# francescobrigante/Audio-Style-Transfer

Measured on AMD Instinct MI355X. Metric: audio-seconds/sec/node (train step, 4s@22.05kHz pairs), higher is better.
Workload: dtype bf16; 1 GPU; configs[1]: batch=8 4 s clips per GPU (S=2, x=(B,S,2,287,597)), full train2 step: STFT + CQT front-end from resident waveforms, encoders+decoder+discriminator, all losses, D and G phases, grad clip, Adam; global_batch=8, parallelism=dp1, hip_graph=True, dp_semantics=per-rank BN and batch-coupled losses

## Files before the change

### audio-style-transfer_amd/ast_amd/_lib.py

```python
from __future__ import annotations

import ctypes as C
import os

import torch

_HERE = os.path.dirname(os.path.abspath(__file__))
LIB_PATH = os.environ.get("AST_HIP_LIB") or os.path.join(_HERE, "libast_hip.so")

F32, BF16 = 0, 1
MAX_TAPS = 9
IGEMM_ACCUMULATE, IGEMM_RELU, IGEMM_WS_ZEROED, IGEMM_STATS, IGEMM_BN_SUMS, IGEMM_BN_NO_RELU, IGEMM_PER_IMAGE = (1 << b for b in range(7))
IGEMM_SLOTS_SHIFT, IGEMM_DET = 8, 4096

vp, i32, i64, f32 = C.c_void_p, C.c_int32, C.c_int64, C.c_float


class Gather(C.Structure):
    _fields_ = [(n, i32) for n in ("N", "Hs", "Ws", "Cs", "Hm", "Wm", "sh", "sw", "oh", "ow", "Hd", "Wd", "Cd",
                                   "dsh", "dsw", "doh", "dow", "ntaps", "wtaps")] + [("tap", i32 * MAX_TAPS)]


class WeightDesc(C.Structure):
    _fields_ = [("w", vp), ("u", vp), ("v", vp), ("sigma", vp), ("scratch", vp), ("wf", vp), ("wb", vp)] + \
# ... 27 lines not shown
    "ast_weight_grads_flush_t": ([vp, vp, i32, vp], i32),
    "ast_dropout_fwd": ([vp, vp, vp, i64, f32, C.c_uint64, vp, vp], i32),
    "ast_weight_grad_unpack": ([vp, i32, vp, vp, vp, vp, vp, i32, i32, i32, i32, i32, i32, i32, vp, vp], i32),
    "ast_chan_stats": ([vp, vp, i32, i32, i32, i32, i32, vp], i32),
    "ast_norm_finalize": ([vp, i32, vp, i32, i32, i32, i32, i32, vp, vp, vp, vp, i32, f32, vp, vp, vp, vp, C.c_long, vp], i32),
    "ast_affine_act": ([vp, vp, vp, vp, vp, vp, vp, i32, i32, i32, i32, i32, vp], i32),
    "ast_bn_apply_fwd": ([vp, vp, vp, vp, i32, C.c_long, vp, vp, vp, vp, vp, vp, f32, vp, vp, f32, vp, vp, i32, i32, i32, i32, i32, i32, vp], i32),
    "ast_bn_apply_bwd": ([vp, vp, vp, vp, vp, vp, i32, C.c_long, vp, vp, vp, vp, vp, vp, vp, vp, vp, vp, vp, vp, vp, vp, i32, i32, i32, i32, i32, i32, vp], i32),
    "ast_norm_bwd_sums": ([vp, vp, vp, vp, vp, i32, i32, i32, i32, i32, i32, vp], i32),
    "ast_norm_bwd_sums_pre": ([vp, vp, vp, vp, vp, i32, i32, i32, i32, i32, i32, vp, vp, vp, vp, vp], i32),
    "ast_norm_bwd_apply_pre": ([vp, vp, vp, vp, vp, vp, vp, vp, i32, i32, i32, i32, i32, vp, vp, vp, vp, vp], i32),
    "ast_norm_bwd_finalize": ([vp, i32, i32, i32, i32, i32, vp, vp, vp, vp, vp, vp, vp, vp, vp, vp, vp, vp, vp], i32),
    "ast_norm_bwd_finalize_n": ([vp, i32, i32, i32, i32, i32, vp, vp, vp, vp, vp, vp, vp, vp, vp, vp, vp, vp, C.c_long, vp], i32),
    "ast_igemm_bn": ([vp, vp, vp, vp, C.POINTER(Gather), i32, i32, vp, C.c_long, vp, vp, vp, vp], i32),
    "ast_norm_bwd_apply": ([vp, vp, vp, vp, vp, vp, vp, vp, i32, i32, i32, i32, i32, vp], i32),
    "ast_layernorm_fwd": ([vp, vp, vp, vp, vp, vp, i32, i32, f32, i32, vp], i32),
    "ast_layernorm_bwd": ([vp, vp, vp, vp, vp, vp, vp, vp, i32, i32, i32, vp], i32),
    "ast_add_drop_ln_fwd": ([vp, vp, vp, vp, vp, vp, vp, vp, vp, i32, i32, f32, f32, C.c_uint64, vp, vp], i32),
    "ast_add_drop_ln_bwd": ([vp, vp, vp, vp, vp, vp, vp, vp, vp, vp, vp, i32, i32, vp], i32),
    "ast_adaptive_pool_fwd": ([vp, vp, i32, i32, i32, i32, i32, i32, i32, vp], i32),
    "ast_adaptive_pool_bwd": ([vp, vp, i32, i32, i32, i32, i32, i32, i32, vp], i32),
    "ast_bilinear_fwd": ([vp, vp, i32, i32, i32, i32, i32, i32, i32, i32, vp], i32),
    "ast_bilinear_bwd": ([vp, vp, i32, i32, i32, i32, i32, i32, i32, i32, vp], i32),
    "ast_attn_fwd": ([vp, vp, vp, vp, vp, i32, i32, i32, i32, i32, i32, i32, i32, i32, vp, vp], i32),
    "ast_attn_bwd": ([vp, vp, vp, vp, vp, vp, vp, vp, i32, i32, i32, i32, i32, i32, i32, i32, vp, vp], i32),
    "ast_rowmix": ([vp, vp, vp, i32, i32, i32, vp], i32),
    "ast_attn_fwd_p": ([vp, vp, vp, vp, vp, i32, i32, i32, i32, i32, i32, i32, i32, i32, vp, f32, C.c_uint64, vp, vp], i32),
    "ast_attn_bwd_p": ([vp, vp, vp, vp, vp, vp, vp, vp, i32, i32, i32, i32, i32, i32, i32, i32, vp, f32, C.c_uint64, vp, vp], i32),
    "ast_add": ([vp, vp, vp, i64, i32, vp], i32),
    "ast_relu_bwd": ([vp, vp, vp, i64, i32, vp], i32),
    "ast_dropout_mask": ([vp, i64, f32, C.c_uint64, vp, vp], i32),
    "ast_mul": ([vp, vp, vp, i64, i32, vp], i32),
    "ast_recon_loss": ([vp, vp, i64, i32, i32, i32, i32, f32, f32, f32, f32, f32, vp, vp, vp], i32),
    "ast_recon_loss_total": ([vp, vp, i64, i32, i32, i32, i32, C.POINTER(f32), C.POINTER(f32), vp, vp, vp, vp], i32),
    "ast_infonce": ([vp, vp, i32, i32, f32, vp, vp, vp, vp], i32),
    "ast_margin": ([vp, i32, i32, f32, vp, vp, vp], i32),
    "ast_hsic": ([vp, vp, i32, i32, vp, vp, vp, vp, vp], i32),
    "ast_crosscov": ([vp, vp, i32, i32, vp, vp, vp, vp, vp], i32),
    "ast_istft": ([vp, i32, i32, vp, vp, vp], i32),
    "ast_bin_stats_acc": ([vp, vp, vp, i32, i32, i32, vp], i32),
    "ast_zscore": ([vp, vp, vp, vp, i32, i32, i32, f32, vp], i32),
    "ast_sections_overlap_avg": ([vp, vp, i32, i32, i32, i32, i32, i32, i32, vp], i32),
    "ast_cross_entropy": ([vp, vp, i32, i32, vp, vp, vp], i32),
    "ast_softmax_entropy": ([vp, i32, i32, vp, vp, vp], i32),
    "ast_scale": ([vp, vp, f32, vp, i64, i32, vp], i32),
    "ast_colsum_acc": ([vp, i64, i32, i32, vp, i32, vp], i32),
    "ast_sumsq": ([vp, i64, vp, vp], i32),
    "ast_adam": ([vp, vp, vp, vp, i64, f32, f32, f32, f32, f32, vp, vp, f32, vp], i32),
    "ast_adam_dev": ([vp, vp, vp, vp, i64, vp, f32, f32, f32, f32, vp, vp, vp], i32),
    "ast_set_values": ([vp, C.POINTER(f32), i32, vp], i32),
    "ast_weighted_sum": ([C.POINTER(vp), C.POINTER(i32), i32, vp, vp, vp], i32),
    "ast_weighted_sum_bwd": ([vp, C.POINTER(i32), i32, vp, vp, vp], i32),
    "ast_counter_incr": ([vp, vp], i32),
    "ast_stft_sections": ([vp, i32, i32, vp, vp, vp, i32, i32, i32, i32, vp], i32),
    "ast_cqt_octaves": ([vp, vp, vp, vp, vp, vp, i32, i32, vp, vp, vp, i32, vp, i32, i32, i32, vp], i32),
    "ast_cqt_sections": ([vp, i32, i32, i32, vp, vp, vp, i32, i32, i32, i32, i32, vp], i32),
    "ast_resample_poly": ([vp, i32, i32, vp, i32, i32, i32, i32, vp, i32, f32, vp], i32),
    "ast_wgrad_rep": ([vp, vp, vp, C.POINTER(Gather), i32, i32, vp], i32),
    "ast_wgrad_slab": ([vp, vp, vp, C.POINTER(Gather), i32, i32, C.POINTER(i32), vp], i32),
    "ast_slab_sum": ([C.POINTER(vp), C.POINTER(i64), C.POINTER(i32), i32, vp], i32),
    "ast_ordered_sum": ([vp, i64, i32, i32, vp, i32, vp], i32),
    "ast_igemm_ws_floats_det": ([C.POINTER(Gather), i32], C.c_long),
    "ast_sumsq_det": ([vp, i64, vp, vp, i32, vp], i32),
    "ast_colsum_acc_det": ([vp, i64, i32, i32, vp, i32, vp, i32, vp], i32),
    "ast_chan_stats_det": ([vp, vp, i32, i32, i32, i32, vp, i32, vp], i32),
    "ast_norm_bwd_sums_det": ([vp, vp, vp, vp, vp, i32, i32, i32, i32, i32, vp, vp, vp, vp, vp, i32, vp], i32),
    "ast_layernorm_bwd_det": ([vp, vp, vp, vp, vp, vp, vp, vp, i32, i32, i32, vp, vp], i32),
    "ast_add_drop_ln_bwd_det": ([vp, vp, vp, vp, vp, vp, vp, vp, vp, vp, vp, i32, i32, vp, vp], i32),
    "ast_recon_loss_total_det": ([vp, vp, i64, i32, i32, i32, i32, C.POINTER(f32), C.POINTER(f32), vp, C.c_long, vp, vp, vp], i32),
    "ast_weight_grads_flush_det": ([vp, vp, i32, vp, C.c_long, vp], i32),
    "ast_bigk_gemm_det_ws_floats": ([i32, i32, i32], C.c_long),
    "ast_bigk_gemm_det": ([vp, vp, vp, vp, i32, i32, i32, vp, C.c_long, vp], i32),
    "ast_bign_dgrad_det_ws_floats": ([i32, i32, i32], C.c_long),
    "ast_bign_dgrad_det": ([vp, vp, vp, i32, i32, i32, i32, vp, C.c_long, vp], i32),
    "ast_skinny_gemm_wide": ([vp, vp, vp, vp, i32, i32, i32, i32, i32, i32, vp], i32),
    "ast_skinny_gemm_wide_ex": ([vp, vp, vp, vp, i32, i32, i32, i32, i32, i32, vp, vp, f32, C.c_uint64, vp, vp], i32),
    "ast_linear_wgrad_wide": ([vp, vp, vp, vp, i32, i32, i32, i32, i32, vp], i32),
    "ast_bigk_gemm_wide": ([vp, vp, vp, vp, i32, i32, i32, i32, vp], i32),
    "ast_bigk_gemm_wide_det_ws_floats": ([i32, i32, i32], C.c_long),
    "ast_bigk_gemm_wide_det": ([vp, vp, vp, vp, i32, i32, i32, vp, C.c_long, vp], i32),
    "ast_bign_dgrad_wide": ([vp, vp, vp, i32, i32, i32, i32, vp], i32),
    "ast_bign_dgrad_wide_det_ws_floats": ([i32, i32, i32], C.c_long),
    "ast_bign_dgrad_wide_det": ([vp, vp, vp, i32, i32, i32, i32, vp, C.c_long, vp], i32),
    "ast_tok_max_ops": ([], i32),
    "ast_tok_program": ([vp, i32, i32, i32, vp, vp, vp, vp], i32),
    "ast_attn_fwd_len": ([vp, vp, vp, vp, vp, i32, i32, i32, i32, i32, i32, i32, i32, i32, vp, i32, vp], i32),
    "ast_sections_overlap_avg_len": ([vp, vp, i32, i32, i32, i32, i32, i32, i32, vp, vp, vp], i32),
    "ast_istft_len": ([vp, i32, i32, vp, vp, vp, vp], i32),
    "ast_frontend_lengths": ([vp, i32, i32, i32, i32, vp, vp, vp], i32),
    "ast_frontend_lengths_host": ([i32, i32, i32, i32, C.POINTER(i32 * 4)], i32),
    "ast_stft_sections_len": ([vp, i32, i32, vp, vp, vp, i32, i32, i32, i32, vp, vp], i32),
    "ast_decimate2_len": ([vp, i32, i32, vp, i32, i32, vp, i32, f32, vp, i32, i32, i32, i32, vp], i32),
    "ast_cqt_octaves_len": ([vp, vp, vp, vp, vp, vp, i32, i32, vp, vp, vp, i32, vp, i32, i32, i32, vp, i32, i32, i32, vp], i32),
    "ast_cqt_sections_len": ([vp, i32, i32, i32, vp, vp, vp, i32, i32, i32, i32, i32, vp, i32, vp], i32),
    "ast_bign_gemm_len": ([vp, vp, vp, vp, i32, i32, i32, i32, i32, i32, vp, vp], i32),
    "ast_resample_poly_len": ([vp, i32, i32, i32, vp, i32, i32, i32, i32, vp, i32, f32, vp, vp, vp], i32),
    "ast_spec_mse_ws_floats": ([i32, i32, i32], C.c_long),
    "ast_spec_mse_len": ([vp, i32, vp, i32, i32, vp, vp, i32, vp, C.c_long, vp, vp], i32),
    "ast_band_energy_ws_floats": ([i32, i32], C.c_long),
    "ast_band_energy_len": ([vp, i32, i32, vp, i32, vp, C.c_long, vp, vp], i32),
    "ast_band_energy_run_frames": ([], i32),
    "ast_pearson_rows": ([vp, vp, i32, i32, vp, vp], i32),
    "ast_mel_table_words": ([], i32),
    "ast_mel_table": ([i32, vp], i32),
    "ast_mfcc_run_frames": ([], i32),
    "ast_mfcc_ws_floats": ([i32, i32, i32], C.c_long),
    "ast_mfcc_len": ([vp, i32, i32, vp, i32, i32, i32, vp, vp, C.c_long, vp, vp], i32),
    "ast_mfcc_distance_ws_floats": ([i32, i32, i32, i32], C.c_long),
    "ast_mfcc_distance_len": ([vp, i32, vp, i32, i32, vp, vp, i32, i32, i32, vp, vp, C.c_long, vp, vp], i32),
    "ast_onset_tile_frames": ([], i32),
    "ast_recurrence_chunk_frames": ([], i32),
    "ast_onset_strength_ws_floats": ([i32, i32], C.c_long),
    "ast_onset_strength_len": ([vp, i32, i32, vp, i32, vp, vp, C.c_long, vp, vp], i32),
    "ast_onset_detect_ws_floats": ([i32, i32], C.c_long),
    "ast_onset_detect_len": ([vp, i32, i32, vp, i32, vp, vp, C.c_long, vp, vp], i32),
    "ast_onset_accuracy_ws_floats": ([i32, i32, i32], C.c_long),
    "ast_onset_accuracy_len": ([vp, i32, vp, i32, i32, vp, vp, i32, vp, vp, C.c_long, vp, vp], i32),
    "ast_recurrence_ws_floats": ([i32, i32], C.c_long),
    "ast_recurrence_len": ([vp, i32, i32, vp, i32, vp, vp, C.c_long, vp, vp, vp], i32),
    "ast_self_similarity_distance_ws_floats": ([i32, i32, i32], C.c_long),
    "ast_self_similarity_distance_len": ([vp, i32, vp, i32, i32, vp, vp, i32, vp, vp, C.c_long, vp, vp], i32),
    "ast_frame_rms_tile_frames": ([], i32),
    "ast_mfcc_mean_chunk_frames": ([], i32),
    "ast_frame_rms_ws_floats": ([i32, i32], C.c_long),
    "ast_frame_rms_len": ([vp, i32, i32, vp, f32, i32, vp, C.c_long, vp, vp, vp, vp, vp, vp, vp], i32),
    "ast_window_sound_len": ([vp, i32, i32, vp, i32, f32, vp, vp, vp], i32),
    "ast_mfcc_mean_ws_floats": ([i32, i32, i32], C.c_long),
    "ast_mfcc_mean_len": ([vp, i32, i32, vp, i32, i32, i32, vp, vp, C.c_long, vp, vp], i32),
    "ast_gain_rows_len": ([vp, i32, i32, vp, vp, C.c_double, vp, vp], i32),
    "ast_chroma_run_frames": ([], i32),
    "ast_pitch_band": ([i32, C.POINTER(i32), C.POINTER(i32)], i32),
    "ast_tuning_debug_words": ([], i32),
    "ast_tuning_ws_floats": ([i32, i32, i32], C.c_long),
    "ast_tuning_len": ([vp, i32, i32, vp, vp, i32, i32, i32, i32, vp, C.c_long, vp, vp, vp], i32),
    "ast_chroma_len": ([vp, i32, i32, vp, vp, i32, i32, i32, i32, vp, vp, vp], i32),
    "ast_chroma_distance_ws_floats": ([i32, i32, i32], C.c_long),
    "ast_chroma_distance_len": ([vp, i32, vp, i32, i32, vp, vp, i32, vp, C.c_long, vp, vp], i32),
    "ast_chroma_similarity_ws_floats": ([i32, i32, i32], C.c_long),
    "ast_chroma_similarity_len": ([vp, i32, vp, i32, i32, vp, vp, i32, vp, C.c_long, vp, vp], i32),
    "ast_pitch_mean_len": ([vp, i32, i32, vp, vp, i32, i32, vp, vp], i32),
    "ast_pitch_correlation_ws_floats": ([i32, i32, i32], C.c_long),
    "ast_pitch_correlation_len": ([vp, i32, vp, i32, i32, vp, vp, i32, vp, C.c_long, vp, vp], i32),
    "ast_state_digest": ([C.POINTER(vp), C.POINTER(C.c_longlong), i32, vp, vp], i32),
}

EXPORTS = tuple(_SIGS) + ("ast_last_error",)

_lib = None


PROFILE_CALLS = None
NEXT_BYTES = None


def _es(dtype_code):
    return 2 if dtype_code == BF16 else 4


CALL_BYTES = {
    "ast_affine_act": lambda a: a[7] * a[8] * a[9] * _es(a[11]) * (2 + (1 if a[3] else 0)),
    "ast_norm_bwd_apply_pre": lambda a: a[8] * a[9] * a[10] * _es(a[12]) * (3 + (2 if a[3] else 0)),
    "ast_norm_bwd_sums_pre": lambda a: a[5] * a[6] * a[7] * _es(a[9]) * (2 + (1 if a[3] else 0)),
    "ast_bn_apply_fwd": lambda a: a[18] * a[19] * a[20] * _es(a[23]) * (2 + (1 if a[1] else 0)),
    "ast_bn_apply_bwd": lambda a: a[22] * a[23] * a[24] * _es(a[27]) * (3 + (2 if a[2] else 0)),
    "ast_chan_stats": lambda a: a[2] * a[3] * a[4] * _es(a[5]),
    "ast_recon_loss": lambda a: 3 * 4 * a[3] * a[4] * 2 * a[5] * a[6],
# ... 86 lines not shown
```

### audio-style-transfer_amd/ast_amd/config.py

```python
import torch

compute_dtype = torch.float32


def set_compute_dtype(dtype):
    global compute_dtype
    if dtype not in (torch.float32, torch.bfloat16):
        raise ValueError("compute dtype must be torch.float32 or torch.bfloat16")
    compute_dtype = dtype


import os as _os
fused_tokens = _os.environ.get("AST_FUSED_TOKENS", "1") != "0"
tok_programs = int(_os.environ.get("AST_TOK_PROGRAMS", "0"))

fused_bn_stats = _os.environ.get("AST_FUSED_BN_STATS", "1") != "0"

bn_mask_from_preact = _os.environ.get("AST_BN_MASK_FROM_PREACT", "1") != "0"

fused_bn_bwd = _os.environ.get("AST_FUSED_BN_BWD", "1") != "0"

wgrad_replicas = int(_os.environ.get("AST_WGRAD_REPLICAS", "8"))

fused_finalize = _os.environ.get("AST_FUSED_FINALIZE", "0") != "0"

wgrad_slabs = int(_os.environ.get("AST_WGRAD_SLABS", "0"))

wgrad_defer = _os.environ.get("AST_WGRAD_DEFER", "1") != "0"
wgrad_defer_streams = int(_os.environ.get("AST_WGRAD_DEFER_STREAMS", "1"))
wgrad_defer_pool = _os.environ.get("AST_WGRAD_DEFER_POOL", "0") != "0"
wgrad_defer_lend = float(_os.environ.get("AST_WGRAD_DEFER_LEND", "1.0"))

deterministic = _os.environ.get("AST_DETERMINISTIC", "0") not in ("", "0")


def check_deterministic_supported(flag, world=1):
    if not flag:
        return
    if tok_programs != 0:
        raise ValueError("deterministic mode: the token programs (AST_TOK_PROGRAMS != 0) add floats with atomics; set AST_TOK_PROGRAMS=0")
    if world > 1:
        raise ValueError("deterministic mode covers one GPU (world == 1); data parallelism is not supported")


def set_deterministic(flag):
    global deterministic
    flag = bool(flag)
    check_deterministic_supported(flag)
    deterministic = flag
```

### audio-style-transfer_amd/ast_amd/decoder_trunk.py

```python
from __future__ import annotations

import torch
import torch.nn as nn

from . import layers as L
from . import config, ops, tokprog
from ._lib import len_tensor
from .style_encoder import SinusoidalPositionalEncoding, _module_bank


def bank_linear(bank, lin: nn.Linear):
    return bank.add(lin.weight, "linear", L.tok_dtype, bias=lin.bias)


class DecoderTrunk(nn.Module):
    token_programs = False

    decode_mode = "recompute"

    def _build_trunk(self, d_model, nhead, num_layers, dim_feedforward, dropout):
        self.d_model = d_model
        self.content_proj = nn.Linear(d_model, d_model)
        self.class_proj = nn.Linear(d_model, d_model)
        self.pos_encoding = SinusoidalPositionalEncoding(d_model)
        layer = nn.TransformerDecoderLayer(d_model=d_model, nhead=nhead, dim_feedforward=dim_feedforward, dropout=dropout,
                                           batch_first=True, norm_first=True)
        self.transformer_decoder = nn.TransformerDecoder(layer, num_layers=num_layers)
        self.start_token = nn.Parameter(torch.randn(1, 1, d_model))
        self.input_norm = nn.LayerNorm(d_model)
        self.output_norm = nn.LayerNorm(d_model)
        self.dropout = nn.Dropout(dropout)

    def _init_weights(self):
        for name, p in self.named_parameters():
            if "weight" in name:
                nn.init.xavier_uniform_(p, gain=0.2) if p.dim() > 1 else nn.init.zeros_(p)
            elif "bias" in name:
                nn.init.zeros_(p)

    def register(self, bank):
        self._cp, self._kp = bank_linear(bank, self.content_proj), bank_linear(bank, self.class_proj)
        self._layers = [L.DecoderLayer(bank, l) for l in self.transformer_decoder.layers]

    def _prepare(self):
        _module_bank(self).prepare(self.training)

    def _check_lengths(self, lengths, B):
        len_tensor(lengths, B, "lengths", training=self.training)

    def _memory(self, content_emb, class_emb):
        B, Sc, D = content_emb.shape
        if 2 * Sc > ops.ATTN_MAX_L:
            raise ValueError(f"{Sc} content sections make {2 * Sc} memory tokens; the attention core takes {ops.ATTN_MAX_L} "
                             f"(at most {ops.ATTN_MAX_L // 2} sections per clip)")
        cm = L.linear(content_emb.reshape(B * Sc, D), self._cp).view(B, Sc, D)
        km = L.linear(class_emb, self._kp).unsqueeze(1).expand(-1, Sc, -1)
        return ops.dropout(torch.cat([cm, km], dim=1), self.dropout.p, self.training)

    def prepare_memory(self, content_emb, class_emb, lengths=None):
        self._check_lengths(lengths, content_emb.shape[0])
        self._prepare()
        return self._memory(content_emb, class_emb)

    def _stack(self, tgt, memory, lengths=None):
        if (self.token_programs and lengths is None and config.tok_programs > 0
                and tokprog.decoder_stack_ok(tgt, memory, self._layers)):
            return tokprog.decoder_stack(tgt, memory, self._layers, self.training)
        for lyr in self._layers:
            tgt = lyr(tgt, memory, self.training, lengths)
        return tgt

    def _teacher_forced(self, emb, memory):
        tgt = torch.cat([self.start_token.expand(emb.shape[0], 1, -1), emb[:, :-1, :]], dim=1)
        tgt = L.layer_norm(self.pos_encoding(tgt), self.input_norm)
        return self._generate(self._stack(tgt, memory), None)

    def forward_training(self, y, memory):
        self._prepare()
        return self._training_pass(y, memory)

    def _inference_pass_cached(self, memory, target_length, lengths=None):
        B = memory.size(0)
        mem_kv = [lyr.memory_kv(memory) for lyr in self._layers]
        caches = [None] * len(self._layers)
        tok = self.start_token.expand(B, -1, -1)
        pe = self.pos_encoding.pe
        outs = []
        for t in range(target_length):
            x = tok + pe[:, t:t + 1]
            for i, lyr in enumerate(self._layers):
                x, caches[i] = lyr.step(x, caches[i], mem_kv[i], lengths)
            outs.append(x)
            tok = x
        return self._generate(torch.cat(outs, dim=1), lengths)

    def _inference_pass(self, memory, target_length=None, lengths=None):
        B = memory.size(0)
        if target_length is None:
            target_length = memory.size(1) // 2
        if target_length > self.pos_encoding.pe.size(1):
            raise ValueError(f"target_length {target_length}, but the positional table holds {self.pos_encoding.pe.size(1)} positions")
        if self.decode_mode == "kv_cache" and not torch.is_grad_enabled():
            return self._inference_pass_cached(memory, target_length, lengths)
        seq = self.start_token.expand(B, -1, -1)
        outs = []
        for _ in range(target_length):
            nxt = self._stack(self.pos_encoding(seq), memory, lengths)[:, -1:, :]
            outs.append(nxt)
            seq = torch.cat([seq, nxt], dim=1)
        return self._generate(torch.cat(outs, dim=1), lengths)

    def forward_inference(self, memory, target_length=None, lengths=None):
        self._check_lengths(lengths, memory.size(0))
        self._prepare()
        return self._inference_pass(memory, target_length, lengths)
```

### audio-style-transfer_amd/ast_amd/layers.py

```python
from __future__ import annotations

import contextlib
import ctypes as C
import os

import torch
import torch.nn as nn

from . import config, ops, streams
from ._lib import LinWg, WeightDesc, check, dcode, lib, ptr, stream
from .ops import PackedWeight, pad8


class WeightBank:

    def __init__(self):
        self.specs = []
        self.entries: list[PackedWeight] = []
        self._key = None
        self._keys = {}
        self._flush_pending = False
        self._flush_stream = None
        self._lin_deferred = []
        self._pinned = []
# ... 353 lines not shown
    return _bn_apply(x, bn, training, relu, stats)


def conv_with_stats(x, pw, k, stride, pad, training):
    stats = None
    if training and config.fused_bn_stats:
        N, H, W, Cs = x.shape
        g, _ = ops.gather_direct(N, H, W, Cs, pw.Cop, k, stride, pad)
        if ops.stats_fusable(g, ops.dcode(x.dtype)):
            stats = ops.stat_table(ops.stat_slots(pw.Cop) * pw.Cop * 2, x.device)
    return ops.Conv2dFn.apply(x, pw.weight, pw, k, stride, pad, False, stats, _link_of(x)), stats


def convT_bn_act(x, pw, k, stride, pad, out_pad, bn: nn.BatchNorm2d, training, relu=True):
    stats = None
    if training and config.fused_bn_stats:
        N, H, W, Cs = x.shape
        Ho = (H - 1) * stride - 2 * pad + k + out_pad
        Wo = (W - 1) * stride - 2 * pad + k + out_pad
        gs = ops.gathers_transposed(N, H, W, Cs, Ho, Wo, pw.Cop, k, stride, pad)
        if all(ops.stats_fusable(g, ops.dcode(x.dtype)) for g in gs):
            stats = ops.stat_table(ops.stat_slots(pw.Cop) * pw.Cop * 2, x.device)
    y = ops.ConvT2dFn.apply(x, pw.weight, pw, k, stride, pad, out_pad, False, stats, _link_of(x))
    return _bn_apply(y, bn, training, relu, stats)


def res_head(x, p1, pd, stride, training):
    stats = None
    if training and config.fused_bn_stats:
        N, H, W, Cs = x.shape
        g, _ = ops.gather_direct(N, H, W, Cs, p1.Cop, 3, stride, 1)
        if ops.stats_fusable(g, ops.dcode(x.dtype)):
            stats = ops.stat_table(ops.stat_slots(p1.Cop) * p1.Cop * 2, x.device)
    in_stats = None
    if training and config.fused_bn_stats:
        N, H, W, Cs = x.shape
        gd, _ = ops.gather_direct(N, H, W, Cs, pd.Cop, 1, stride, 0)
        if ops.in_stats_fusable(gd, ops.dcode(x.dtype)):
            in_stats = ops.stat_table(N * pd.Cop * 2, x.device)
    c1, idn = ops.ResHeadFn.apply(x, p1.weight, pd.weight, p1, pd, stride, stats, in_stats)
    return c1, idn, stats, in_stats


def conv_bn_act(x, pw, k, stride, pad, bn: nn.BatchNorm2d, training, relu=True):
    y, stats = conv_with_stats(x, pw, k, stride, pad, training)
    return _bn_apply(y, bn, training, relu, stats)


def layer_norm(x, ln: nn.LayerNorm):
    return ops.LayerNormFn.apply(x, ln.weight, ln.bias, ln.eps)


class MHA:

    def __init__(self, bank: WeightBank, m: nn.MultiheadAttention, cross: bool):
        d = m.embed_dim
        self.m, self.d, self.h, self.cross = m, d, m.num_heads, cross
        if cross:
            self.q = bank.add(m.in_proj_weight, "linear", tok_dtype, bias=m.in_proj_bias, rows=(0, d))
            self.kv = bank.add(m.in_proj_weight, "linear", tok_dtype, bias=m.in_proj_bias, rows=(d, 3 * d))
        else:
            self.qkv = bank.add(m.in_proj_weight, "linear", tok_dtype, bias=m.in_proj_bias)
        self.out = bank.add(m.out_proj.weight, "linear", tok_dtype, bias=m.out_proj.bias)

    def __call__(self, x, mem, training, p_drop, causal=False, key_mask=None):
        B, Lq, d = x.shape
        dh = d // self.h
        if self.cross:
            Lk = mem.shape[1]
            q = linear(x.reshape(B * Lq, d), self.q)
            kv = linear(mem.reshape(B * Lk, d), self.kv)
            k_off, v_off = 0, d
        else:
            Lk = Lq
            q = kv = linear(x.reshape(B * Lq, d), self.qkv)
            k_off, v_off = d, 2 * d
        if key_mask is not None:
            ops.require_inference(q, kv)
        o = ops.AttnCoreFn.apply(q, kv, B, self.h, Lq, Lk, dh, k_off, v_off, causal, float(p_drop) if training else 0.0,
                                 *(key_mask or ()))
        return linear(o, self.out).view(B, Lq, d)


class EncoderLayer:

    def __init__(self, bank, layer: nn.TransformerEncoderLayer):
        self.l = layer
        self.attn = MHA(bank, layer.self_attn, cross=False)
        self.ff1 = bank.add(layer.linear1.weight, "linear", tok_dtype, bias=layer.linear1.bias)
        self.ff2 = bank.add(layer.linear2.weight, "linear", tok_dtype, bias=layer.linear2.bias)

    def __call__(self, x, training, lengths=None):
        l, p = self.l, self.l.dropout.p
        B, L, d = x.shape
        km = None if lengths is None else (lengths, L)
        if not config.fused_tokens:
            x = layer_norm(x + ops.dropout(self.attn(x, None, training, l.self_attn.dropout, key_mask=km), l.dropout1.p, training),
                           l.norm1)
            h = ops.dropout(linear(x.reshape(B * L, d), self.ff1, relu=True), p, training)
            h = ops.dropout(linear(h, self.ff2), l.dropout2.p, training).view(B, L, d)
            return layer_norm(x + h, l.norm2)
        _, x = ops.add_drop_ln(x, self.attn(x, None, training, l.self_attn.dropout, key_mask=km), l.norm1, l.dropout1.p, training)
        h = ops.ffn(x.reshape(B * L, d), self.ff1, self.ff2, p, training)
        _, y = ops.add_drop_ln(x, h.view(B, L, d), l.norm2, l.dropout2.p, training)
        return y


class DecoderLayer:

    def __init__(self, bank, layer: nn.TransformerDecoderLayer):
        self.l = layer
        self.sa = MHA(bank, layer.self_attn, cross=False)
        self.ca = MHA(bank, layer.multihead_attn, cross=True)
        self.ff1 = bank.add(layer.linear1.weight, "linear", tok_dtype, bias=layer.linear1.bias)
        self.ff2 = bank.add(layer.linear2.weight, "linear", tok_dtype, bias=layer.linear2.bias)

    def __call__(self, x, memory, training, lengths=None):
        l = self.l
        B, L, d = x.shape
        km = None if lengths is None else (lengths, memory.shape[1] // 2)
        if not config.fused_tokens:
            h = layer_norm(x, l.norm1)
            x = x + ops.dropout(self.sa(h, None, training, l.self_attn.dropout, causal=True), l.dropout1.p, training)
            h = layer_norm(x, l.norm2)
            x = x + ops.dropout(self.ca(h, memory, training, l.multihead_attn.dropout, key_mask=km), l.dropout2.p, training)
            h = layer_norm(x, l.norm3)
            h = ops.dropout(linear(h.reshape(B * L, d), self.ff1, relu=True), l.dropout.p, training)
            h = ops.dropout(linear(h, self.ff2), l.dropout3.p, training).view(B, L, d)
            return x + h
        h = layer_norm(x, l.norm1)
        x, h = ops.add_drop_ln(x, self.sa(h, None, training, l.self_attn.dropout, causal=True), l.norm2, l.dropout1.p, training)
        x, h = ops.add_drop_ln(x, self.ca(h, memory, training, l.multihead_attn.dropout, key_mask=km), l.norm3, l.dropout2.p, training)
        h = ops.ffn(h.reshape(B * L, d), self.ff1, self.ff2, l.dropout.p, training)
        x, _ = ops.add_drop_ln(x, h.view(B, L, d), None, l.dropout3.p, training)
        return x

    def memory_kv(self, memory):
        B, Lm, d = memory.shape
        return linear(memory.reshape(B * Lm, d), self.ca.kv), Lm

    def step(self, x_t, kv_self, mem_kv, lengths=None):
        l = self.l
        B, _, d = x_t.shape
        dh = d // self.sa.h
        h = layer_norm(x_t, l.norm1).reshape(B, d)
        qkv = linear(h, self.sa.qkv)
        new_kv = qkv[:, d:].reshape(B, 1, 2 * d)
        kv_self = new_kv if kv_self is None else torch.cat([kv_self, new_kv], dim=1)
        t1 = kv_self.shape[1]
        q = qkv[:, :d].contiguous()
        o = ops.AttnCoreFn.apply(q, kv_self.reshape(B * t1, 2 * d), B, self.sa.h, 1, t1, dh, 0, d, False, 0.0)
        x = x_t.reshape(B, d) + linear(o, self.sa.out)
        h = layer_norm(x, l.norm2)
        kvm, Lm = mem_kv
        qm = linear(h, self.ca.q)
        if lengths is not None:
            ops.require_inference(qm, kvm)
        o = ops.AttnCoreFn.apply(qm, kvm, B, self.ca.h, 1, Lm, dh, 0, d, False, 0.0, *(() if lengths is None else (lengths, Lm // 2)))
        x = x + linear(o, self.ca.out)
        h = layer_norm(x, l.norm3)
        x = x + linear(linear(h, self.ff1, relu=True), self.ff2)
        return x.view(B, 1, d), kv_self
```

### audio-style-transfer_amd/ast_amd/ops.py

```python
from __future__ import annotations

import ctypes
import functools
import math

import torch

from . import _lib, config
from ._lib import Gather, check, dcode, len_tensor, lib, ptr, stream


@functools.lru_cache(maxsize=None)
def const_tensor(values, dtype, device):
    return torch.tensor(values, dtype=dtype, device=device)


def pad8(c: int) -> int:
    return (c + 7) // 8 * 8


def _tap(dh, dw, wt):
    return (dh + 64) | ((dw + 64) << 8) | (wt << 16)


# ... 313 lines not shown
        _igemm(x, pwd.wf, pwd.bias_ptr_tensor(), idn, gd, stats=in_stats, per_image=in_stats is not None)
        ctx.save_for_backward(x)
        ctx.pws, ctx.geoms, ctx.stride = (pw1, pwd), (g1, gd), stride
        return c1, idn

    @staticmethod
    def backward(ctx, dc1, didn):
        (x,) = ctx.saved_tensors
        (pw1, pwd), (g1, gd), stride = ctx.pws, ctx.geoms, ctx.stride
        dc1, didn = dc1.contiguous(), didn.contiguous()
        N, H, W, Cs = x.shape
        if pw1.dwp is None or pwd.dwp is None:
            raise RuntimeError("weights were prepared in eval/no-grad mode; run the forward in training mode before backward")
        _wgrad(dc1, x, pw1.dwp, g1, pw1.replicas, pw1)
        _wgrad(didn, x, pwd.dwp, gd, pwd.replicas, pwd)
        pw1.bank.request_flush()
        dx = None
        if ctx.needs_input_grad[0]:
            dx = torch.empty_like(x)
            Ho, Wo = dc1.shape[1], dc1.shape[2]
            for g in gathers_transposed(N, Ho, Wo, pw1.Cop, H, W, Cs, 3, stride, 1):
                _igemm(dc1, pw1.wb, None, dx, g)
            for g in gathers_transposed(N, Ho, Wo, pwd.Cop, H, W, Cs, 1, stride, 0):
                if g.ntaps > 0:
                    _igemm(didn, pwd.wb, None, dx, g, flags=_lib.IGEMM_ACCUMULATE)
        return dx, None, None, None, None, None, None, None


class ConvT2dFn(torch.autograd.Function):

    @staticmethod
    def forward(ctx, x, weight, pw: PackedWeight, k, stride, pad, out_pad, bias_grad, stats=None, link=None):
        N, H, W, Cs = x.shape
        Ho = (H - 1) * stride - 2 * pad + k + out_pad
        Wo = (W - 1) * stride - 2 * pad + k + out_pad
        y = torch.empty((N, Ho, Wo, pw.Cop), dtype=x.dtype, device=x.device)
        b = pw.bias_ptr_tensor()
        for g in gathers_transposed(N, H, W, Cs, Ho, Wo, pw.Cop, k, stride, pad):
            _igemm(x, pw.wf, b, y, g, stats=stats)
        ctx.save_for_backward(x)
        ctx.pw, ctx.args, ctx.bias_grad, ctx.link = pw, (k, stride, pad, Ho, Wo), bias_grad, link
        return y

    @staticmethod
    def backward(ctx, dy):
        (x,) = ctx.saved_tensors
        pw, (k, stride, pad, Ho, Wo) = ctx.pw, ctx.args
        dy = dy.contiguous()
        N, H, W, Cs = x.shape
        g, (Hx, Wx) = gather_direct(N, Ho, Wo, pw.Cop, Cs, k, stride, pad)
        assert (Hx, Wx) == (H, W), "ConvTranspose2d geometry mismatch"
        if pw.dwp is None:
            raise RuntimeError("weights were prepared in eval/no-grad mode; run the forward in training mode before backward")
        _wgrad(x, dy, pw.dwp, g, pw.replicas, pw)
        pw.bank.request_flush()
        if ctx.bias_grad:
            pw.add_bias_grad(dy)
        dx = None
        if ctx.needs_input_grad[0]:
            dx = torch.empty_like(x)
            link = _bn_link_ready(ctx.link, (g,), x)
            _igemm(dy, pw.wb, None, dx, g, bn=link)
            if link is not None:
                link.filled = True
        return dx, None, None, None, None, None, None, None, None, None


SKINNY_MAX_ROWS = 64
WIDE_MAX_ROWS = 1024
ATTN_MAX_L = 1024


def _token_entry(who, stem, rows, tail=""):
    if rows > WIDE_MAX_ROWS:
        raise RuntimeError(f"{who}: {rows} token rows > {WIDE_MAX_ROWS} (the cap of the wide token path, AST_WIDE_MAX_ROWS)")
    return f"ast_{stem}{'' if rows <= SKINNY_MAX_ROWS else '_wide'}{tail}"


def _token_call(who, stem, rows, tail, *args):
    name = _token_entry(who, stem, rows, tail)
    check(getattr(lib(), name)(*args, stream()), name)


def _token_rows_ok(rows):
    return rows <= SKINNY_MAX_ROWS or (config.deterministic and rows <= WIDE_MAX_ROWS)


class LinearFn(torch.autograd.Function):

    @staticmethod
    def forward(ctx, x, weight, pw: PackedWeight, relu):
        x = x.contiguous()
        rows = x.shape[0]
        assert x.shape[1] == pw.Cip and x.dtype == pw.dtype, (x.shape, pw.Cip, x.dtype, pw.dtype)
        ctx.skinny = (_token_rows_ok(rows) and pw.KK == 1 and pw.u is None and pw.Ci == pw.Cip
                      and (rows <= SKINNY_MAX_ROWS or x.dtype == torch.float32))
        y = torch.empty((rows, pw.Cop), dtype=x.dtype, device=x.device)
        if ctx.skinny:
            if pw.Cop != pw.Co:
                y.zero_()
            b = None if pw.bias is None else pw.bias.data_ptr() + 4 * pw.b_off
            _token_call("LinearFn", "skinny_gemm", rows, "", ptr(x), pw.weight.data_ptr() + 4 * pw.w_off, b, ptr(y), rows, pw.Co, pw.Ci, pw.s_co, pw.Cop, int(relu))
        else:
            g, _ = gather_direct(rows, 1, 1, pw.Cip, pw.Cop, 1, 1, 0)
            _igemm(x, pw.wf, pw.bias_ptr_tensor(), y, g, _lib.IGEMM_RELU if relu else 0)
        ctx.save_for_backward(x, y if relu else None)
        ctx.pw, ctx.relu = pw, relu
        return y

    @staticmethod
    def backward(ctx, dy):
        x, y = ctx.saved_tensors
        pw = ctx.pw
        dy = dy.contiguous()
        rows = x.shape[0]
        if ctx.relu:
            dz = torch.empty_like(dy)
            check(lib().ast_relu_bwd(ptr(dy), ptr(y), ptr(dz), dy.numel(), dcode(dy.dtype), stream()), "ast_relu_bwd")
            dy = dz
        dx = None
        if ctx.skinny:
            if pw.bank is not None:
                pw.bank.defer_linear_wgrad(pw, dy, x)
            else:
                gw = acc_grad(pw.weight)
                gb = None if pw.bias is None else acc_grad(pw.bias).data_ptr() + 4 * pw.b_off
                _token_call("LinearFn", "linear_wgrad", rows, "", ptr(dy), ptr(x), gw.data_ptr() + 4 * pw.w_off, gb, rows, pw.Co, pw.Ci, pw.Cop, pw.s_co)
            if ctx.needs_input_grad[0]:
                dx = torch.empty_like(x)
                _token_call("LinearFn", "skinny_gemm", rows, "", ptr(dy), ptr(pw.wb), None, ptr(dx), rows, pw.Ci, pw.Cop, pw.Cop, pw.Cip, 0)
            return dx, None, None, None
        if config.deterministic:
            raise RuntimeError(f"LinearFn: the non-skinny weight gradient (> {WIDE_MAX_ROWS} token rows, spectral norm, unpadded channels "
                               "or bf16 above 64 rows) has no deterministic form")
        g, _ = gather_direct(rows, 1, 1, pw.Cip, pw.Cop, 1, 1, 0)
        dwp = torch.zeros((pw.Cop, 1, pw.Cip), dtype=torch.float32, device=x.device)
        _wgrad(dy, x, dwp, g)
        pw.add_weight_grad(dwp, 0)
        pw.add_bias_grad(dy)
        if ctx.needs_input_grad[0]:
            gb, _ = gather_direct(rows, 1, 1, pw.Cop, pw.Cip, 1, 1, 0)
            dx = torch.empty_like(x)
            _igemm(dy, pw.wb, None, dx, gb)
        return dx, None, None, None


class BigLinearFn(torch.autograd.Function):

    @staticmethod
    def forward(ctx, x, weight, bias):
        x = x.contiguous()
        rows, K = x.shape
        N = weight.shape[0]
        assert weight.shape[1] == K and x.dtype == torch.float32 and weight.is_contiguous()
        ctx.big_in = K > N
        stem, tail = ("bigk_gemm", "_det" if config.deterministic else "") if ctx.big_in else ("skinny_gemm", "")
        _token_entry("BigLinearFn", stem, rows, tail)
        y = torch.empty((rows, N), dtype=torch.float32, device=x.device)
        if tail:
            ws = det_ws(getattr(lib(), _token_entry("BigLinearFn", stem, rows, "_det_ws_floats"))(rows, N, K), x.device)
            _token_call("BigLinearFn", stem, rows, tail, ptr(x), ptr(weight), ptr(bias), ptr(y), rows, N, K, ptr(ws), ws.numel())
        elif ctx.big_in:
            _token_call("BigLinearFn", stem, rows, tail, ptr(x), ptr(weight), ptr(bias), ptr(y), rows, N, K, N)
        else:
            _token_call("BigLinearFn", stem, rows, tail, ptr(x), ptr(weight), ptr(bias), ptr(y), rows, N, K, K, N, 0)
        ctx.save_for_backward(x)
        ctx.weight, ctx.bias = weight, bias
        return y

    @staticmethod
    def backward(ctx, dy):
        (x,) = ctx.saved_tensors
        w, b = ctx.weight, ctx.bias
        dy = dy.contiguous()
        rows, K = x.shape
        N = w.shape[0]
        _token_call("BigLinearFn", "linear_wgrad", rows, "", ptr(dy), ptr(x), ptr(acc_grad(w)), ptr(acc_grad(b)) if b is not None else None, rows, N, K, N, K)
        dx = None
        if ctx.needs_input_grad[0]:
            if ctx.big_in:
                raise NotImplementedError("BigLinearFn: input gradient of the huge-input linear (its input is data on the reference's path)")
            dx = torch.empty_like(x)
            if config.deterministic:
                ws = det_ws(getattr(lib(), _token_entry("BigLinearFn", "bign_dgrad", rows, "_det_ws_floats"))(rows, N, K), x.device)
                _token_call("BigLinearFn", "bign_dgrad", rows, "_det", ptr(dy), ptr(w), ptr(dx), rows, N, K, N, ptr(ws), ws.numel())
            else:
                _token_call("BigLinearFn", "bign_dgrad", rows, "", ptr(dy), ptr(w), ptr(dx), rows, N, K, N)
        return dx, None, None


BIGN_MAX_ROWS = 4096


def big_out_linear(x, weight, bias, S, lengths=None):
    if torch.is_grad_enabled() and any(t is not None and t.requires_grad for t in (x, weight, bias)):
        raise RuntimeError("the length-masked output linear (big_out_linear) is inference only: it has no backward; "
                           "run it under torch.no_grad()")
    x = x.contiguous()
    rows, K = x.shape
    N = weight.shape[0]
    assert weight.shape[1] == K and x.dtype == torch.float32 and weight.dtype == torch.float32 and weight.is_contiguous()
    if rows > BIGN_MAX_ROWS:
        raise RuntimeError(f"big_out_linear: {rows} rows > {BIGN_MAX_ROWS} (AST_BIGN_MAX_ROWS)")
    if S < 1 or rows % S:
        raise ValueError(f"big_out_linear: {rows} rows are not a whole number of clips of {S} sections")
    lengths = len_tensor(lengths, rows // S, "lengths", contiguous=True)
    y = torch.empty((rows, N), dtype=torch.float32, device=x.device)
    check(lib().ast_bign_gemm_len(ptr(x), ptr(weight), ptr(bias), ptr(y), rows, N, K, K, N, int(S), ptr(lengths), stream()),
          "ast_bign_gemm_len")
    return y


class FFNFn(torch.autograd.Function):

    @staticmethod
    def forward(ctx, x, w1, w2, pw1: PackedWeight, pw2: PackedWeight, p):
        x = x.contiguous()
        rows = x.shape[0]
        h = torch.empty((rows, pw1.Cop), dtype=x.dtype, device=x.device)
        y = torch.empty((rows, pw2.Cop), dtype=x.dtype, device=x.device)
        mask, seed, ctr = None, 0, None
        if p > 0.0:
            if _DropState.counter is None or _DropState.counter.device != x.device:
                _DropState.counter = torch.zeros(1, dtype=torch.int64, device=x.device)
            _DropState.calls += 1
            seed, ctr = _DropState.seed + 7919 * _DropState.calls, _DropState.counter
            mask = torch.empty_like(h)
        _token_call("FFNFn", "skinny_gemm", rows, "_ex", ptr(x), pw1.weight.data_ptr() + 4 * pw1.w_off, pw1.bias.data_ptr() + 4 * pw1.b_off, ptr(h),
                                                 rows, pw1.Co, pw1.Ci, pw1.s_co, pw1.Cop, 1, None, ptr(mask), float(p), seed, ptr(ctr))
        _token_call("FFNFn", "skinny_gemm", rows, "", ptr(h), pw2.weight.data_ptr() + 4 * pw2.w_off, pw2.bias.data_ptr() + 4 * pw2.b_off, ptr(y),
                                          rows, pw2.Co, pw2.Ci, pw2.s_co, pw2.Cop, 0)
        ctx.save_for_backward(x, h, mask)
        ctx.pw1, ctx.pw2 = pw1, pw2
        return y

    @staticmethod
    def backward(ctx, dy):
        x, h, mask = ctx.saved_tensors
        pw1, pw2 = ctx.pw1, ctx.pw2
        dy = dy.contiguous()
        rows = x.shape[0]
        pw2.bank.defer_linear_wgrad(pw2, dy, h)
        dh = torch.empty_like(h)
        if mask is None:
            _token_call("FFNFn", "skinny_gemm", rows, "", ptr(dy), ptr(pw2.wb), None, ptr(dh), rows, pw2.Ci, pw2.Cop, pw2.Cop, pw2.Cip, 0)
            dz = torch.empty_like(dh)
            check(lib().ast_relu_bwd(ptr(dh), ptr(h), ptr(dz), dh.numel(), dcode(dh.dtype), stream()), "ast_relu_bwd")
            dh = dz
        else:
            _token_call("FFNFn", "skinny_gemm", rows, "_ex", ptr(dy), ptr(pw2.wb), None, ptr(dh), rows, pw2.Ci, pw2.Cop, pw2.Cop, pw2.Cip, 0, ptr(mask), None,
                                                     0.0, 0, None)
        pw1.bank.defer_linear_wgrad(pw1, dh, x)
        dx = None
        if ctx.needs_input_grad[0]:
            dx = torch.empty_like(x)
            _token_call("FFNFn", "skinny_gemm", rows, "", ptr(dh), ptr(pw1.wb), None, ptr(dx), rows, pw1.Ci, pw1.Cop, pw1.Cop, pw1.Cip, 0)
        return dx, None, None, None, None, None


def _skinny_ok(pw, rows):
    return (_token_rows_ok(rows) and pw.KK == 1 and pw.u is None and pw.Ci == pw.Cip and pw.Co == pw.Cop and pw.bank is not None
            and pw.bias is not None)


def ffn(x2d, pw1, pw2, p, training):
    rows = x2d.shape[0]
    if _skinny_ok(pw1, rows) and _skinny_ok(pw2, rows) and x2d.dtype == torch.float32:
        return FFNFn.apply(x2d, pw1.weight, pw2.weight, pw1, pw2, float(p) if training else 0.0)
    h = dropout(LinearFn.apply(x2d, pw1.weight, pw1, True), p, training)
    h = h if pw1.Cop == pw1.Co else h[:, :pw1.Co]
    y = LinearFn.apply(h, pw2.weight, pw2, False)
    return y if pw2.Cop == pw2.Co else y[:, :pw2.Co]


_scratch = {}


def _clean_scratch(n, device, tag=None):
    key = (n, device, torch.cuda.current_stream(device).cuda_stream, tag)
    t = _scratch.get(key)
    if t is None:
        t = _scratch[key] = torch.zeros(n, dtype=torch.float32, device=device)
    return t


def det_slots(rows, per=1):
    return max(1, min(512 // per, (int(rows) + 255) // 256))


def det_ws(n, device):
    return _clean_scratch(max(1, int(n)), device, tag="det")


def _stats(x):
    N, H, W, C = x.shape
    sums = stat_table(N * C * 2, x.device)
    if config.deterministic:
        ns = det_slots(H * W, N)
        check(lib().ast_chan_stats_det(ptr(x), ptr(sums), N, H * W, C, dcode(x.dtype), ptr(det_ws(N * ns * C * 2, x.device)), ns, stream()),
              "ast_chan_stats_det")
        return sums
    check(lib().ast_chan_stats(ptr(x), ptr(sums), N, H * W, C, dcode(x.dtype), 1, stream()), "ast_chan_stats")
    return sums


def _bwd_sums(dy, y, x, r, sums3, N, HW, C, relu, dt, scale1, shift1, scale2, shift2):
    y, r, scale1, shift1, scale2, shift2 = (t if (t is None or isinstance(t, int)) else ptr(t) for t in (y, r, scale1, shift1, scale2, shift2))
    if config.deterministic:
        ns = det_slots(HW, N)
        check(lib().ast_norm_bwd_sums_det(ptr(dy), y, ptr(x), r, ptr(sums3), N, HW, C, int(relu), dt, scale1, shift1,
                                          scale2, shift2, ptr(det_ws(N * ns * C * 3, dy.device)), ns, stream()), "ast_norm_bwd_sums_det")
        return
    check(lib().ast_norm_bwd_sums_pre(ptr(dy), y, ptr(x), r, ptr(sums3), N, HW, C, int(relu), dt, 1,
                                      scale1, shift1, scale2, shift2, stream()), "ast_norm_bwd_sums")


class _SyncBN:
    world = 1
    group = None
    active = False


def set_sync_bn(world=1, group=None, force=False):
    _SyncBN.world, _SyncBN.group = int(world), group
    _SyncBN.active = _SyncBN.world > 1 or bool(force)


def _global_sums(sums, n_floats):
    import torch.distributed as dist
    g = sums[:n_floats].clone()
    dist.all_reduce(g, op=dist.ReduceOp.SUM, group=_SyncBN.group)
    return g


def _bn_batch_stats(x, gamma, beta, bn, stats=None):
    N, H, W, C = x.shape
    rows = stats.numel() // (2 * C) if stats is not None else N
    sums = stats if stats is not None else _stats(x)
    pixels = N * H * W
# ... 111 lines not shown
        N, H, W, C = c2.shape
        Creal = g1.numel()
        ctx.fused = bool(training and config.fused_finalize and not _SyncBN.active)
        if ctx.fused:
            tab1 = stats if stats is not None else _stats(c2)
            tab2 = in_stats if in_stats is not None else _stats(ds)
            rows1 = tab1.numel() // (2 * C)
            out1 = torch.empty((4, C), dtype=torch.float32, device=c2.device)
            out2 = torch.empty((4, N * C), dtype=torch.float32, device=c2.device)
            y = torch.empty_like(c2)
            check(lib().ast_bn_apply_fwd(ptr(c2), ptr(ds), ptr(y), ptr(tab1), rows1, N * H * W, ptr(tab2), ptr(g1), ptr(b1), ptr(bn.running_mean),
                                         ptr(bn.running_var), ptr(bn.num_batches_tracked), bn.eps, ptr(g2), ptr(b2), inn.eps, ptr(out1), ptr(out2),
                                         N, H * W, C, Creal, 1, dcode(c2.dtype), stream()), "ast_bn_apply_fwd")
            ctx.save_for_backward(c2, ds, None, out1[0], out1[1], out2[0], out2[1], out1[2], out1[3], out2[2], out2[3])
            ctx.params, ctx.training = (g1, b1, g2, b2), training
            return y
        if training:
            m1, r1, s1, f1 = _bn_batch_stats(c2, g1, b1, bn, stats)
        else:
            m1, r1, s1, f1 = _finalize(None, N, H * W, C, Creal, False, g1, b1, bn.running_mean, bn.running_var,
                                       True, bn.eps, c2.device)
        m2, r2, s2, f2 = _finalize(in_stats if in_stats is not None else _stats(ds), N, H * W, C, Creal, True, g2, b2, None, None, False,
                                   inn.eps, c2.device)
        y = torch.empty_like(c2)
        check(lib().ast_affine_act(ptr(c2), ptr(s1), ptr(f1), ptr(ds), ptr(s2), ptr(f2), ptr(y), N, H * W, C, 1,
                                   dcode(c2.dtype), stream()), "ast_affine_act")
        ctx.save_for_backward(c2, ds, y, m1, r1, m2, r2, s1, f1, s2, f2)
        ctx.params, ctx.training = (g1, b1, g2, b2), training
        return y

    @staticmethod
    def backward(ctx, dy):
        c2, ds, y, m1, r1, m2, r2, s1, f1, s2, f2 = ctx.saved_tensors
        pre = config.bn_mask_from_preact
        if not ctx.training:
            raise RuntimeError("ResTailFn: backward in eval mode is not on the reference's path")
        g1, b1, g2, b2 = ctx.params
        dy = dy.contiguous()
        N, H, W, C = c2.shape
        dev = c2.device
        if ctx.fused:
            tab3 = stat_table(N * C * 3, dev)
            _bwd_sums(dy, None, c2, ds, tab3, N, H * W, C, 1, dcode(c2.dtype), s1, f1, s2, f2)
            dc2, dds = torch.empty_like(c2), torch.empty_like(ds)
            check(lib().ast_bn_apply_bwd(ptr(dy), ptr(c2), ptr(ds), ptr(dc2), ptr(dds), ptr(tab3), N, N * H * W, ptr(g1), ptr(m1), ptr(r1),
                                         ptr(acc_grad(g1)), ptr(acc_grad(b1)), ptr(g2), ptr(m2), ptr(r2), ptr(acc_grad(g2)), ptr(acc_grad(b2)),
                                         ptr(s1), ptr(f1), ptr(s2), ptr(f2), N, H * W, C, g1.numel(), 1, dcode(c2.dtype), stream()), "ast_bn_apply_bwd")
            return dc2, dds, None, None, None, None, None, None, None, None, None
        sums3 = _clean_scratch(N * C * 3, dev)
        coef = (ptr(s1), ptr(f1), ptr(s2), ptr(f2)) if pre else (None, None, None, None)
        _bwd_sums(dy, y, c2, ds, sums3, N, H * W, C, 1, dcode(c2.dtype), *coef)
        k1 = torch.empty((C, 3), dtype=torch.float32, device=dev)
        k2 = torch.empty((N, C, 3), dtype=torch.float32, device=dev)
        gsum = _global_sums(sums3, N * C * 3) if _SyncBN.active else None
        check(lib().ast_norm_bwd_finalize(ptr(sums3), 1, N, H * W, C, g1.numel(), ptr(g1), ptr(m1), ptr(r1),
                                          ptr(acc_grad(g1)), ptr(acc_grad(b1)), ptr(k1), ptr(g2), ptr(m2), ptr(r2),
                                          ptr(acc_grad(g2)), ptr(acc_grad(b2)), ptr(k2), stream()),
              "ast_norm_bwd_finalize")
        if gsum is not None:
            check(lib().ast_norm_bwd_finalize(ptr(gsum), 0, N, H * W * _SyncBN.world, C, g1.numel(), ptr(g1), ptr(m1), ptr(r1),
                                              None, None, ptr(k1), None, None, None, None, None, None, stream()), "ast_norm_bwd_finalize")
        dc2, dds = torch.empty_like(c2), torch.empty_like(ds)
        check(lib().ast_norm_bwd_apply_pre(ptr(dy), ptr(y), ptr(c2), ptr(ds), ptr(k1), ptr(k2), ptr(dc2), ptr(dds), N, H * W,
                                           C, 1, dcode(c2.dtype), *coef, stream()), "ast_norm_bwd_apply")
        return dc2, dds, None, None, None, None, None, None, None, None, None


class LayerNormFn(torch.autograd.Function):
    @staticmethod
    def forward(ctx, x, gamma, beta, eps):
        shape = x.shape
        x2 = x.contiguous().view(-1, shape[-1])
        rows, D = x2.shape
        y = torch.empty_like(x2)
        mean = torch.empty(rows, dtype=torch.float32, device=x.device)
        rstd = torch.empty_like(mean)
        check(lib().ast_layernorm_fwd(ptr(x2), ptr(gamma), ptr(beta), ptr(y), ptr(mean), ptr(rstd), rows, D, eps,
                                      dcode(x2.dtype), stream()), "ast_layernorm_fwd")
        ctx.save_for_backward(x2, mean, rstd)
        ctx.gamma, ctx.beta, ctx.shape = gamma, beta, shape
        return y.view(shape)

    @staticmethod
    def backward(ctx, dy):
        x2, mean, rstd = ctx.saved_tensors
        rows, D = x2.shape
        dy2 = dy.contiguous().view(rows, D)
        dx = torch.empty_like(x2)
        if config.deterministic:
            check(lib().ast_layernorm_bwd_det(ptr(dy2), ptr(x2), ptr(ctx.gamma), ptr(mean), ptr(rstd), ptr(dx), ptr(acc_grad(ctx.gamma)),
                                              ptr(acc_grad(ctx.beta)), rows, D, dcode(x2.dtype), ptr(det_ws(2 * rows * D, dx.device)),
                                              stream()), "ast_layernorm_bwd_det")
            return dx.view(ctx.shape), None, None, None
        check(lib().ast_layernorm_bwd(ptr(dy2), ptr(x2), ptr(ctx.gamma), ptr(mean), ptr(rstd), ptr(dx),
                                      ptr(acc_grad(ctx.gamma)), ptr(acc_grad(ctx.beta)), rows, D, dcode(x2.dtype),
                                      stream()), "ast_layernorm_bwd")
        return dx.view(ctx.shape), None, None, None


class AddDropLNFn(torch.autograd.Function):

    @staticmethod
    def forward(ctx, x, sub, ln, p):
        ctx.set_materialize_grads(False)
        shape = sub.shape
        D = shape[-1]
        sub2 = sub.contiguous().view(-1, D)
        x2 = x.contiguous().view(-1, D) if x is not None else None
        rows = sub2.shape[0]
        s = torch.empty_like(sub2)
        mask = torch.empty_like(sub2) if p > 0.0 else None
        seed = 0
        if p > 0.0:
            if _DropState.counter is None or _DropState.counter.device != sub.device:
                _DropState.counter = torch.zeros(1, dtype=torch.int64, device=sub.device)
            _DropState.calls += 1
            seed = _DropState.seed + 7919 * _DropState.calls
        y = mean = rstd = None
        if ln is not None:
            y = torch.empty_like(sub2)
            mean = torch.empty(rows, dtype=torch.float32, device=sub.device)
            rstd = torch.empty_like(mean)
        check(lib().ast_add_drop_ln_fwd(ptr(x2), ptr(sub2), ptr(mask), ptr(s), ptr(ln.weight) if ln is not None else None,
                                        ptr(ln.bias) if ln is not None else None, ptr(y), ptr(mean), ptr(rstd), rows, D,
                                        float(ln.eps) if ln is not None else 0.0, float(p), seed,
                                        ptr(_DropState.counter) if p > 0.0 else None, stream()), "ast_add_drop_ln_fwd")
        ctx.save_for_backward(s, mean, rstd, mask)
        ctx.ln, ctx.shape, ctx.has_x = ln, shape, x is not None
        if ln is None:
            return s.view(shape)
        return s.view(shape), y.view(shape)

    @staticmethod
    def backward(ctx, ds_ext, dy=None):
        s, mean, rstd, mask = ctx.saved_tensors
        rows, D = s.shape
        if ds_ext is None and dy is None:
            return None, None, None, None
        ds2 = ds_ext.contiguous().view(rows, D) if ds_ext is not None else None
        dy2 = dy.contiguous().view(rows, D) if dy is not None else None
        want_dx = ctx.has_x and ctx.needs_input_grad[0]
        dx = None if (not want_dx or dy2 is None) else torch.empty_like(s)
        if dy2 is None and mask is None:
            return (ds_ext if want_dx else None), ds_ext, None, None
        dsub = torch.empty_like(s)
        ln = ctx.ln
        if config.deterministic:
            check(lib().ast_add_drop_ln_bwd_det(ptr(dy2), ptr(ds2), ptr(s), ptr(ln.weight) if dy2 is not None else None, ptr(mean),
                                                ptr(rstd), ptr(mask), ptr(dx), ptr(dsub),
                                                ptr(acc_grad(ln.weight)) if dy2 is not None else None,
                                                ptr(acc_grad(ln.bias)) if dy2 is not None else None, rows, D,
                                                ptr(det_ws(2 * rows * D, dsub.device)), stream()), "ast_add_drop_ln_bwd_det")
        else:
            check(lib().ast_add_drop_ln_bwd(ptr(dy2), ptr(ds2), ptr(s), ptr(ln.weight) if dy2 is not None else None, ptr(mean), ptr(rstd),
                                            ptr(mask), ptr(dx), ptr(dsub), ptr(acc_grad(ln.weight)) if dy2 is not None else None,
                                            ptr(acc_grad(ln.bias)) if dy2 is not None else None, rows, D, stream()), "ast_add_drop_ln_bwd")
        if want_dx and dx is None:
            dx = ds2
        return (dx.view(ctx.shape) if want_dx else None), dsub.view(ctx.shape), None, None


def add_drop_ln(x, sub, ln, p, training):
    out = AddDropLNFn.apply(x, sub, ln, float(p) if training else 0.0)
    return (out, None) if ln is None else out


class RowMixFn(torch.autograd.Function):

    @staticmethod
    def forward(ctx, x, A, At):
        x = x.contiguous()
        R_out, R_in = A.shape
        assert x.shape[0] == R_in and x.dtype == torch.float32
        y = torch.empty((R_out, x.shape[1]), dtype=torch.float32, device=x.device)
        check(lib().ast_rowmix(ptr(A), ptr(x), ptr(y), R_out, R_in, x.shape[1], stream()), "ast_rowmix")
        ctx.At = At
        return y

    @staticmethod
# ... 441 lines not shown
```

### audio-style-transfer_amd/csrc/ast_common.h

```cpp
#pragma once
#include <hip/hip_runtime.h>
#include <stdint.h>
#include <stdio.h>
#include <stdlib.h>
#include <string.h>
#include <algorithm>
#include <atomic>
#include <initializer_list>

typedef __bf16 bf16_t;
typedef __attribute__((ext_vector_type(8))) __bf16 bf16x8;
typedef __attribute__((ext_vector_type(4))) __bf16 bf16x4;
typedef __attribute__((ext_vector_type(4))) float f32x4;
typedef __attribute__((ext_vector_type(2))) float f32x2;

enum { AST_F32 = 0, AST_BF16 = 1 };

void ast_set_error(const char* fmt, ...);
#define AST_FAIL(...) do { ast_set_error(__VA_ARGS__); return -1; } while (0)
#define AST_CHECK_LAUNCH() do { hipError_t e_ = hipGetLastError(); \
    if (e_ != hipSuccess) { ast_set_error("%s:%d launch failed: %s", __FILE__, __LINE__, hipGetErrorString(e_)); return -2; } } while (0)
#define AST_HIP(x) do { hipError_t e_ = (x); \
    if (e_ != hipSuccess) { ast_set_error("%s:%d %s: %s", __FILE__, __LINE__, #x, hipGetErrorString(e_)); return -3; } } while (0)

// ... 10 lines not shown
    for (const void* k : kernels) AST_HIP(hipFuncSetAttribute(k, hipFuncAttributeMaxDynamicSharedMemorySize, bytes));
    if (tracked) done[dev].store(true, std::memory_order_release);
    return 0;
  }
};

template <typename T> struct U8;
template <> struct U8<float> {
  static __device__ __forceinline__ void load(const float* p, float (&v)[8]) {
    f32x4 a = *reinterpret_cast<const f32x4*>(p);
    f32x4 b = *reinterpret_cast<const f32x4*>(p + 4);
#pragma unroll
    for (int i = 0; i < 4; ++i) { v[i] = a[i]; v[4 + i] = b[i]; }
  }
  static __device__ __forceinline__ void store(float* p, const float (&v)[8]) {
    f32x4 a, b;
#pragma unroll
    for (int i = 0; i < 4; ++i) { a[i] = v[i]; b[i] = v[4 + i]; }
    *reinterpret_cast<f32x4*>(p) = a;
    *reinterpret_cast<f32x4*>(p + 4) = b;
  }
};
template <> struct U8<bf16_t> {
  static __device__ __forceinline__ void load(const bf16_t* p, float (&v)[8]) {
    bf16x8 a = *reinterpret_cast<const bf16x8*>(p);
#pragma unroll
    for (int i = 0; i < 8; ++i) v[i] = (float)a[i];
  }
  static __device__ __forceinline__ void store(bf16_t* p, const float (&v)[8]) {
    bf16x8 a;
#pragma unroll
    for (int i = 0; i < 8; ++i) a[i] = (bf16_t)v[i];
    *reinterpret_cast<bf16x8*>(p) = a;
  }
};

template <int CTRL>
__device__ __forceinline__ float dpp_mov(float v) {
  return __builtin_bit_cast(float, __builtin_amdgcn_update_dpp(0, __builtin_bit_cast(int, v), CTRL, 0xF, 0xF, false));
}
__device__ __forceinline__ float row16_sum(float v) {
  v += dpp_mov<0xB1>(v);
  v += dpp_mov<0x4E>(v);
  v += dpp_mov<0x124>(v);
  v += dpp_mov<0x128>(v);
  return v;
}
__device__ __forceinline__ float row16_transpose_sum(const float (&v)[16], const int l) {
  float w[8], x[4], y[2];
  const bool b0 = l & 1, b1 = l & 2, b2 = l & 4, b3 = l & 8;
#pragma unroll
  for (int k = 0; k < 8; ++k) w[k] = (b0 ? v[2 * k + 1] : v[2 * k]) + dpp_mov<0xB1>(b0 ? v[2 * k] : v[2 * k + 1]);
#pragma unroll
  for (int k = 0; k < 4; ++k) x[k] = (b1 ? w[2 * k + 1] : w[2 * k]) + dpp_mov<0x4E>(b1 ? w[2 * k] : w[2 * k + 1]);
#pragma unroll
  for (int k = 0; k < 2; ++k) {
    const float send = b2 ? x[2 * k] : x[2 * k + 1];
    const float lo = dpp_mov<0x124>(send), hi = dpp_mov<0x12C>(send);
    y[k] = (b2 ? x[2 * k + 1] : x[2 * k]) + (b2 ? lo : hi);
  }
  return (b3 ? y[1] : y[0]) + dpp_mov<0x128>(b3 ? y[0] : y[1]);
}
__device__ __forceinline__ float wave_sum_dpp(float v) {
  v = row16_sum(v);
  const int i = __builtin_bit_cast(int, v);
  return (__builtin_bit_cast(float, __builtin_amdgcn_readlane(i, 0)) + __builtin_bit_cast(float, __builtin_amdgcn_readlane(i, 16))) +
         (__builtin_bit_cast(float, __builtin_amdgcn_readlane(i, 32)) + __builtin_bit_cast(float, __builtin_amdgcn_readlane(i, 48)));
}
#ifdef AST_WAVE_SUM_SHFL
__device__ __forceinline__ float wave_sum(float v) {
#pragma unroll
  for (int o = 32; o > 0; o >>= 1) v += __shfl_xor(v, o, 64);
  return v;
}
#else
__device__ __forceinline__ float wave_sum(float v) { return wave_sum_dpp(v); }
#endif
__device__ __forceinline__ float wave_max(float v) {
#pragma unroll
  for (int o = 32; o > 0; o >>= 1) v = fmaxf(v, __shfl_xor(v, o, 64));
  return v;
}

__device__ __forceinline__ uint64_t mix64(uint64_t z) {
  z += 0x9E3779B97F4A7C15ull; z = (z ^ (z >> 30)) * 0xBF58476D1CE4E5B9ull; z = (z ^ (z >> 27)) * 0x94D049BB133111EBull; return z ^ (z >> 31);
}
__device__ __forceinline__ float dropout_keep(uint64_t base, uint64_t i, float p, float keep) {
  const uint32_t r = (uint32_t)(mix64(base + i) >> 40);
  return ((float)r * (1.f / 16777216.f)) >= p ? keep : 0.f;
}

__device__ __forceinline__ float block_sum(float v, float* red ) {
  v = wave_sum(v);
  const int w = threadIdx.x >> 6, nw = (blockDim.x + 63) >> 6;
  __syncthreads();
  if ((threadIdx.x & 63) == 0) red[w] = v;
  __syncthreads();
  if (threadIdx.x == 0) { float s = 0.f; for (int i = 0; i < nw; ++i) s += red[i]; red[16] = s; }
  __syncthreads();
  return red[16];
}

#define AST_DISPATCH_T(dtype, ...) \
  do { if ((dtype) == AST_F32) { using T = float; __VA_ARGS__; } \
       else if ((dtype) == AST_BF16) { using T = bf16_t; __VA_ARGS__; } \
       else AST_FAIL("%s: bad dtype %d", __func__, (int)(dtype)); } while (0)

#define AST_HIDDEN __attribute__((visibility("hidden")))
AST_HIDDEN int attn_long_fwd_launch(const float* q, const float* k, const float* v, float* o, float* probs, int B, int H, int Lq, int Lk,
                                    int dh, int ldq, int ldk, int ldo, int causal, const float* drop_mask, float p, uint64_t seed,
                                    const int64_t* d_offset, void* stream);
AST_HIDDEN int attn_long_fwd_len_launch(const float* q, const float* k, const float* v, float* o, float* probs, int B, int H, int Lq,
                                        int Lk, int dh, int ldq, int ldk, int ldo, int causal, const int32_t* key_len, int key_period,
                                        void* stream);
AST_HIDDEN int attn_long_bwd_launch(const float* dout, const float* q, const float* k, const float* v, const float* probs, float* dq,
                                    float* dk, float* dv, int B, int H, int Lq, int Lk, int dh, int ldq, int ldk, int ldo,
                                    const float* drop_mask, float p, uint64_t seed, const int64_t* d_offset, void* stream);
```

### audio-style-transfer_amd/csrc/norm.hip

```cpp
#include "ast_common.h"
#include "../../include/ast_hip.h"

namespace {

template <typename T, int MODE, bool DET = false>
__global__ __launch_bounds__(256) void chan_reduce_kernel(const T* __restrict__ a, const T* __restrict__ b,
                                                           const T* __restrict__ c, const T* __restrict__ d,
                                                           float* __restrict__ sums, int HW, int C, int ppb, int relu,
                                                           const float* __restrict__ sc1, const float* __restrict__ sf1,
                                                           const float* __restrict__ sc2, const float* __restrict__ sf2) {
  constexpr int K = MODE == 0 ? 2 : 3;
  __shared__ float red[256 * 8];
  const int U = C >> 3;
  const int PL = 256 / U;
  const int tid = threadIdx.x;
  const int u = tid % U, pl = tid / U;
  const int n = blockIdx.y;
  const int p0 = blockIdx.x * ppb, p1 = min(HW, p0 + ppb);
  float s[K][8];
#pragma unroll
  for (int k = 0; k < K; ++k)
#pragma unroll
    for (int i = 0; i < 8; ++i) s[k][i] = 0.f;
  float a1[8], b1[8], a2[8], b2[8];
// ... 418 lines not shown
            dg += (float)((double)rstd2[iq] * ((double)t2 - (double)mean2[iq] * (double)t0));
            db += t0;
          }
          if (dgamma2) dgamma2[c] += dg;
          if (dbeta2) dbeta2[c] += db;
        }
      } else { kc[3 * C + c * 3] = kc[3 * C + c * 3 + 1] = kc[3 * C + c * 3 + 2] = 0.f; }
    }
  }
  __syncthreads();

  const int U = C >> 3;
  const size_t per_img = (size_t)HW * U, base = (size_t)n * per_img;
  const size_t stride = (size_t)gridDim.x * 256;
  const bool hoist = (256 % U) == 0;
  const bool remask = relu != 0;
  float a1[8], b1[8], a2[8], b2[8];
  f32x4 kaq[6], kbq[6];
  auto load_coef = [&](int u) __attribute__((always_inline)) {
    if (remask) {
      U8<float>::load(sc1 + u * 8, a1);
      U8<float>::load(sf1 + u * 8, b1);
      if (r) {
        U8<float>::load(sc2 + (size_t)n * C + u * 8, a2);
        U8<float>::load(sf2 + (size_t)n * C + u * 8, b2);
      }
    }
    const f32x4* ka4 = reinterpret_cast<const f32x4*>(kc + u * 24);
    const f32x4* kb4 = reinterpret_cast<const f32x4*>(kc + 3 * C + u * 24);
#pragma unroll
    for (int q = 0; q < 6; ++q) { kaq[q] = ka4[q]; kbq[q] = dr ? kb4[q] : f32x4{0.f, 0.f, 0.f, 0.f}; }
  };
#define KA(k, q) kaq[((k) * 3 + (q)) >> 2][((k) * 3 + (q)) & 3]
#define KB(k, q) kbq[((k) * 3 + (q)) >> 2][((k) * 3 + (q)) & 3]
  const size_t j0 = (size_t)blockIdx.x * 256 + tid;
  if (hoist) load_coef((int)(j0 % U));
  for (size_t j = j0; j < per_img; j += stride) {
    if (!hoist) load_coef((int)(j % U));
    const size_t i = base + j;
    float dz[8], v[8], o[8], vr[8];
    U8<T>::load(dy + i * 8, dz);
    U8<T>::load(x + i * 8, v);
    if (r) U8<T>::load(r + i * 8, vr);
    if (remask) {
      float pre[8];
#pragma unroll
      for (int k = 0; k < 8; ++k) pre[k] = __builtin_fmaf(v[k], a1[k], b1[k]);
      if (r) {
#pragma unroll
        for (int k = 0; k < 8; ++k) pre[k] += __builtin_fmaf(vr[k], a2[k], b2[k]);
      }
#pragma unroll
      for (int k = 0; k < 8; ++k) dz[k] = pre[k] > 0.f ? dz[k] : 0.f;
    }
#pragma unroll
    for (int k = 0; k < 8; ++k) o[k] = KA(k, 0) * dz[k] + KA(k, 1) * v[k] + KA(k, 2);
    U8<T>::store(dx + i * 8, o);
    if (dr) {
#pragma unroll
      for (int k = 0; k < 8; ++k) o[k] = KB(k, 0) * dz[k] + KB(k, 1) * vr[k] + KB(k, 2);
      U8<T>::store(dr + i * 8, o);
    }
  }
#undef KA
#undef KB
}

__global__ void layernorm_fwd_kernel(const float* __restrict__ x, const float* __restrict__ gamma,
                                     const float* __restrict__ beta, float* __restrict__ y, float* __restrict__ mean,
                                     float* __restrict__ rstd, int rows, int D, float eps) {
  const int row = blockIdx.x * (blockDim.x >> 6) + (threadIdx.x >> 6), lane = threadIdx.x & 63;
  if (row >= rows) return;
  const float* xr = x + (size_t)row * D;
  float s = 0.f;
  for (int i = lane; i < D; i += 64) s += xr[i];
  const float m = wave_sum(s) / D;
  float q = 0.f;
  for (int i = lane; i < D; i += 64) { const float d = xr[i] - m; q += d * d; }
  const float r = rsqrtf(wave_sum(q) / D + eps);
  for (int i = lane; i < D; i += 64) y[(size_t)row * D + i] = (xr[i] - m) * r * gamma[i] + beta[i];
  if (lane == 0) { mean[row] = m; rstd[row] = r; }
}

template <bool DET = false>
__global__ void layernorm_bwd_kernel(const float* __restrict__ dy, const float* __restrict__ x,
                                     const float* __restrict__ gamma, const float* __restrict__ mean,
                                     const float* __restrict__ rstd, float* __restrict__ dx, float* dgamma, float* dbeta,
                                     int rows, int D) {
  const int row = blockIdx.x * (blockDim.x >> 6) + (threadIdx.x >> 6), lane = threadIdx.x & 63;
  if (row >= rows) return;
  const float m = mean[row], r = rstd[row];
  const float* xr = x + (size_t)row * D;
  const float* dr = dy + (size_t)row * D;
  float a = 0.f, b = 0.f;
  for (int i = lane; i < D; i += 64) {
    const float xh = (xr[i] - m) * r, g = dr[i] * gamma[i];
    a += g; b += g * xh;
  }
  a = wave_sum(a) / D; b = wave_sum(b) / D;
  for (int i = lane; i < D; i += 64) {
    const float xh = (xr[i] - m) * r, g = dr[i] * gamma[i];
    dx[(size_t)row * D + i] = r * (g - a - xh * b);
    if constexpr (DET) {
      if (dgamma) dgamma[(size_t)row * D + i] = dr[i] * xh;
      if (dbeta) dbeta[(size_t)row * D + i] = dr[i];
    } else {
      if (dgamma) unsafeAtomicAdd(dgamma + i, dr[i] * xh);
      if (dbeta) unsafeAtomicAdd(dbeta + i, dr[i]);
    }
  }
}


__global__ void add_drop_ln_fwd_kernel(const float* __restrict__ x, const float* __restrict__ sub, float* __restrict__ mask,
                                       float* __restrict__ s_out, const float* __restrict__ gamma, const float* __restrict__ beta,
                                       float* __restrict__ y, float* __restrict__ mean, float* __restrict__ rstd, int rows, int D,
                                       float eps, float p, uint64_t seed, const int64_t* __restrict__ d_offset) {
  const int row = blockIdx.x * (blockDim.x >> 6) + (threadIdx.x >> 6), lane = threadIdx.x & 63;
  if (row >= rows) return;
  const size_t o = (size_t)row * D;
  const uint64_t base = p > 0.f ? mix64(seed ^ mix64((uint64_t)(d_offset ? *d_offset : 0))) : 0;
  const float keep = 1.f / (1.f - p);
  float acc = 0.f;
  for (int i = lane; i < D; i += 64) {
    float v = sub[o + i];
    if (p > 0.f) { const float m = dropout_keep(base, o + i, p, keep); mask[o + i] = m; v *= m; }
    if (x) v += x[o + i];
    s_out[o + i] = v;
    acc += v;
  }
  if (!gamma) return;
  const float m = wave_sum(acc) / D;
  float q = 0.f;
  for (int i = lane; i < D; i += 64) { const float d = s_out[o + i] - m; q += d * d; }
  const float r = rsqrtf(wave_sum(q) / D + eps);
  for (int i = lane; i < D; i += 64) y[o + i] = (s_out[o + i] - m) * r * gamma[i] + beta[i];
  if (lane == 0) { mean[row] = m; rstd[row] = r; }
}

template <bool DET = false>
__global__ void add_drop_ln_bwd_kernel(const float* __restrict__ dy, const float* __restrict__ ds_ext, const float* __restrict__ s,
                                       const float* __restrict__ gamma, const float* __restrict__ mean, const float* __restrict__ rstd,
                                       const float* __restrict__ mask, float* __restrict__ dx, float* __restrict__ dsub,
                                       float* dgamma, float* dbeta, int rows, int D) {
  const int row = blockIdx.x * (blockDim.x >> 6) + (threadIdx.x >> 6), lane = threadIdx.x & 63;
  if (row >= rows) return;
  const size_t o = (size_t)row * D;
  float a = 0.f, b = 0.f, m = 0.f, r = 0.f;
  if (dy) {
    m = mean[row]; r = rstd[row];
    for (int i = lane; i < D; i += 64) {
      const float xh = (s[o + i] - m) * r, g = dy[o + i] * gamma[i];
      a += g; b += g * xh;
    }
    a = wave_sum(a) / D; b = wave_sum(b) / D;
  }
  for (int i = lane; i < D; i += 64) {
    float d = ds_ext ? ds_ext[o + i] : 0.f;
    if (dy) {
      const float xh = (s[o + i] - m) * r, g = dy[o + i] * gamma[i];
      d += r * (g - a - xh * b);
      if constexpr (DET) {
        if (dgamma) dgamma[o + i] = dy[o + i] * xh;
        if (dbeta) dbeta[o + i] = dy[o + i];
      } else {
        if (dgamma) unsafeAtomicAdd(dgamma + i, dy[o + i] * xh);
        if (dbeta) unsafeAtomicAdd(dbeta + i, dy[o + i]);
      }
    }
    if (dx) dx[o + i] = d;
    dsub[o + i] = mask ? d * mask[o + i] : d;
  }
}

__global__ __launch_bounds__(256) void add_drop_ln_fwd256_kernel(const float* __restrict__ x, const float* __restrict__ sub,
                                                                 float* __restrict__ mask, float* __restrict__ s_out,
                                                                 const float* __restrict__ gamma, const float* __restrict__ beta,
                                                                 float* __restrict__ y, float* __restrict__ mean, float* __restrict__ rstd,
                                                                 int rows, float eps, float p, uint64_t seed,
                                                                 const int64_t* __restrict__ d_offset) {
  constexpr int D = 256;
  const int row = blockIdx.x * 4 + (threadIdx.x >> 6), lane = threadIdx.x & 63;
  if (row >= rows) return;
  const size_t o = (size_t)row * D + lane * 4;
  const f32x4 z = {0.f, 0.f, 0.f, 0.f};
  const f32x4 sv = *reinterpret_cast<const f32x4*>(sub + o);
  const f32x4 xv = x ? *reinterpret_cast<const f32x4*>(x + o) : z;
  const f32x4 g4 = gamma ? *reinterpret_cast<const f32x4*>(gamma + lane * 4) : z;
  const f32x4 b4 = gamma ? *reinterpret_cast<const f32x4*>(beta + lane * 4) : z;
  const uint64_t base = p > 0.f ? mix64(seed ^ mix64((uint64_t)(d_offset ? *d_offset : 0))) : 0;
  __builtin_amdgcn_sched_barrier(0);
  const float keep = 1.f / (1.f - p);
  f32x4 sv2 = sv;
  if (p > 0.f) {
    f32x4 m4;
#pragma unroll
    for (int e = 0; e < 4; ++e) { m4[e] = dropout_keep(base, o + e, p, keep); sv2[e] *= m4[e]; }
    *reinterpret_cast<f32x4*>(mask + o) = m4;
  }
  f32x4 s4;
#pragma unroll
  for (int e = 0; e < 4; ++e) s4[e] = x ? sv2[e] + xv[e] : sv2[e];
  *reinterpret_cast<f32x4*>(s_out + o) = s4;
  if (!gamma) return;
  const float m = wave_sum(s4[0] + s4[1] + s4[2] + s4[3]) / D;
  float q = 0.f;
#pragma unroll
  for (int e = 0; e < 4; ++e) { const float d = s4[e] - m; q += d * d; }
  const float r = rsqrtf(wave_sum(q) / D + eps);
  f32x4 y4;
#pragma unroll
  for (int e = 0; e < 4; ++e) y4[e] = (s4[e] - m) * r * g4[e] + b4[e];
  *reinterpret_cast<f32x4*>(y + o) = y4;
  if (lane == 0) { mean[row] = m; rstd[row] = r; }
}

__global__ __launch_bounds__(256) void add_drop_ln_bwd256_kernel(const float* __restrict__ dy, const float* __restrict__ ds_ext,
                                                                 const float* __restrict__ s, const float* __restrict__ gamma,
                                                                 const float* __restrict__ mean, const float* __restrict__ rstd,
                                                                 const float* __restrict__ mask, float* __restrict__ dx,
                                                                 float* __restrict__ dsub, float* dgamma, float* dbeta, int rows) {
  constexpr int D = 256;
  __shared__ float red[2][4][D];
  const int wave = threadIdx.x >> 6, lane = threadIdx.x & 63;
  const int row = blockIdx.x * 4 + wave;
  const bool valid = row < rows;
  const size_t o = (size_t)(valid ? row : 0) * D + lane * 4;
  const f32x4 z = {0.f, 0.f, 0.f, 0.f};
  const f32x4 dy4 = dy ? *reinterpret_cast<const f32x4*>(dy + o) : z;
  const f32x4 s4 = dy ? *reinterpret_cast<const f32x4*>(s + o) : z;
  const f32x4 g4 = dy ? *reinterpret_cast<const f32x4*>(gamma + lane * 4) : z;
  const f32x4 e4 = ds_ext ? *reinterpret_cast<const f32x4*>(ds_ext + o) : z;
  const f32x4 k4 = mask ? *reinterpret_cast<const f32x4*>(mask + o) : f32x4{1.f, 1.f, 1.f, 1.f};
  const float m = dy ? mean[valid ? row : 0] : 0.f, r = dy ? rstd[valid ? row : 0] : 0.f;
  __builtin_amdgcn_sched_barrier(0);
  f32x4 d4 = e4, xh4 = z;
  if (dy) {
    float a = 0.f, b = 0.f;
#pragma unroll
    for (int e = 0; e < 4; ++e) { xh4[e] = (s4[e] - m) * r; const float g = dy4[e] * g4[e]; a += g; b += g * xh4[e]; }
    a = wave_sum(a) / D; b = wave_sum(b) / D;
#pragma unroll
    for (int e = 0; e < 4; ++e) d4[e] += r * (dy4[e] * g4[e] - a - xh4[e] * b);
  }
  if (valid) {
    if (dx) *reinterpret_cast<f32x4*>(dx + o) = d4;
    f32x4 ds4;
#pragma unroll
    for (int e = 0; e < 4; ++e) ds4[e] = d4[e] * k4[e];
    *reinterpret_cast<f32x4*>(dsub + o) = ds4;
  }
  if (dy && (dgamma || dbeta)) {
#pragma unroll
    for (int e = 0; e < 4; ++e) {
      red[0][wave][lane * 4 + e] = valid ? dy4[e] * xh4[e] : 0.f;
      red[1][wave][lane * 4 + e] = valid ? dy4[e] : 0.f;
    }
    __syncthreads();
    const int i = threadIdx.x;
    if (dgamma) unsafeAtomicAdd(dgamma + i, red[0][0][i] + red[0][1][i] + red[0][2][i] + red[0][3][i]);
    if (dbeta) unsafeAtomicAdd(dbeta + i, red[1][0][i] + red[1][1][i] + red[1][2][i] + red[1][3][i]);
  }
}

int reduce_blocks() { static const int v = env_int("AST_REDUCE_BLOCKS", 512); return v; }

int elem_blocks() { static const int v = env_int("AST_ELEM_BLOCKS", 2048); return v; }

int grid_for(size_t n, int block = 256) { return (int)std::min<size_t>((n + block - 1) / block, 256 * 16); }

}

extern "C" int ast_chan_stats(const void* x, float* sums, int N, int HW, int C, int dtype, int assume_zeroed, void* stream) {
  if (!x || !sums || N <= 0 || HW <= 0 || C <= 0 || (C & 7) || C > 2048) AST_FAIL("ast_chan_stats: bad args N=%d HW=%d C=%d", N, HW, C);
  hipStream_t s = (hipStream_t)stream;
  if (!assume_zeroed) AST_HIP(hipMemsetAsync(sums, 0, sizeof(float) * (size_t)N * C * 2, s));
  const int PL = 256 / (C >> 3);
  const int nblk = max(1, min((HW + PL - 1) / PL, max(1, reduce_blocks() / N)));
  const int ppb = (HW + nblk - 1) / nblk;
  dim3 grid((HW + ppb - 1) / ppb, N);
  const float* nf = nullptr;
  AST_DISPATCH_T(dtype, hipLaunchKernelGGL((chan_reduce_kernel<T, 0>), grid, dim3(256), 0, s, (const T*)x, (const T*)nullptr,
                                            (const T*)nullptr, (const T*)nullptr, sums, HW, C, ppb, 0, nf, nf, nf, nf));
  AST_CHECK_LAUNCH();
  return 0;
}

extern "C" int ast_norm_finalize(float* sums, int zero_sums, int64_t* num_batches_tracked, int N, int HW, int C, int Creal, int instance,
                                 const float* gamma, const float* beta, float* running_mean, float* running_var, int eval_mode, float eps,
                                 float* mean, float* rstd, float* scale, float* shift, long count, void* stream) {
  if (!gamma || !beta || !mean || !rstd || !scale || !shift) AST_FAIL("ast_norm_finalize: null pointer");
  if (!eval_mode && !sums) AST_FAIL("ast_norm_finalize: sums required in training mode");
  if (eval_mode && (instance || !running_mean || !running_var)) AST_FAIL("ast_norm_finalize: eval mode needs running stats");
  const int total = instance ? N * C : C;
  hipLaunchKernelGGL(norm_finalize_kernel, dim3((total + 3) / 4), dim3(256), 0, (hipStream_t)stream, sums, zero_sums,
                     num_batches_tracked, N, HW, C, Creal, instance, gamma, beta, running_mean, running_var, eval_mode, eps, mean, rstd,
                     scale, shift, count);
  AST_CHECK_LAUNCH();
  return 0;
}

extern "C" int ast_affine_act(const void* x, const float* scale, const float* shift, const void* r, const float* scale2,
                              const float* shift2, void* y, int N, int HW, int C, int relu, int dtype, void* stream) {
  if (!x || !scale || !shift || !y || (C & 7) || (r && (!scale2 || !shift2))) AST_FAIL("ast_affine_act: bad args");
  const size_t units = (size_t)N * HW * (C >> 3);
  const int s1_per_n = (relu >> 1) & 1;
  const dim3 agrid(std::max(1, std::min<int>((int)(((size_t)HW * (C >> 3) + 255) / 256), std::max(1, elem_blocks() / N))), N);
  AST_DISPATCH_T(dtype, hipLaunchKernelGGL((affine_act_kernel<T>), agrid, dim3(256), 0, (hipStream_t)stream,
                                            (const T*)x, scale, shift, (const T*)r, scale2, shift2, (T*)y, HW, C, units,
                                            s1_per_n, relu & 1));
  AST_CHECK_LAUNCH();
  return 0;
}

extern "C" int ast_norm_bwd_sums_pre(const void* dy, const void* y, const void* x, const void* r, float* sums3, int N, int HW,
                                     int C, int relu, int dtype, int assume_zeroed, const float* scale1, const float* shift1,
                                     const float* scale2, const float* shift2, void* stream) {
  if (!dy || !x || !sums3 || (relu && !y && !scale1) || (C & 7) || C > 2048) AST_FAIL("ast_norm_bwd_sums: bad args");
  if (scale1 && (!shift1 || (r && (!scale2 || !shift2)))) AST_FAIL("ast_norm_bwd_sums: incomplete pre-activation coefficients");
  hipStream_t s = (hipStream_t)stream;
  if (!assume_zeroed) AST_HIP(hipMemsetAsync(sums3, 0, sizeof(float) * (size_t)N * C * 3, s));
  const int PL = 256 / (C >> 3);
  const int nblk = max(1, min((HW + PL - 1) / PL, max(1, reduce_blocks() / N)));
  const int ppb = (HW + nblk - 1) / nblk;
  dim3 grid((HW + ppb - 1) / ppb, N);
  AST_DISPATCH_T(dtype, hipLaunchKernelGGL((chan_reduce_kernel<T, 1>), grid, dim3(256), 0, s, (const T*)dy, (const T*)y,
                                            (const T*)x, (const T*)r, sums3, HW, C, ppb, relu, scale1, shift1, scale2, shift2));
  AST_CHECK_LAUNCH();
  return 0;
}

extern "C" int ast_norm_bwd_sums(const void* dy, const void* y, const void* x, const void* r, float* sums3, int N, int HW,
// ... 9 lines not shown
  hipLaunchKernelGGL(norm_bwd_finalize_kernel, dim3((C + 3) / 4), dim3(256), 0, (hipStream_t)stream, sums3, zero_sums, N, HW, C, Creal,
                     gamma1, mean1, rstd1, dgamma1, dbeta1, k1, gamma2, mean2, rstd2, dgamma2, dbeta2, k2, count);
  AST_CHECK_LAUNCH();
  return 0;
}

extern "C" int ast_norm_bwd_finalize(float* sums3, int zero_sums, int N, int HW, int C, int Creal, const float* gamma1,
                                     const float* mean1, const float* rstd1, float* dgamma1, float* dbeta1, float* k1,
                                     const float* gamma2, const float* mean2, const float* rstd2, float* dgamma2,
                                     float* dbeta2, float* k2, void* stream) {
  return ast_norm_bwd_finalize_n(sums3, zero_sums, N, HW, C, Creal, gamma1, mean1, rstd1, dgamma1, dbeta1, k1, gamma2, mean2, rstd2,
                                 dgamma2, dbeta2, k2, 0, stream);
}

extern "C" int ast_norm_bwd_apply_pre(const void* dy, const void* y, const void* x, const void* r, const float* k1,
                                      const float* k2, void* dx, void* dr, int N, int HW, int C, int relu, int dtype,
                                      const float* scale1, const float* shift1, const float* scale2, const float* shift2,
                                      void* stream) {
  if (!dy || (relu && !y && !scale1) || (dx && k1 && !x) || (dr && (!r || !k2)) || (C & 7)) AST_FAIL("ast_norm_bwd_apply: bad args");
  if (scale1 && (!x || !shift1 || (r && (!scale2 || !shift2)))) AST_FAIL("ast_norm_bwd_apply: incomplete pre-activation coefficients");
  const size_t units = (size_t)N * HW * (C >> 3);
  const dim3 bgrid(std::max(1, std::min<int>((int)(((size_t)HW * (C >> 3) + 255) / 256), std::max(1, elem_blocks() / N))), N);
  AST_DISPATCH_T(dtype, hipLaunchKernelGGL((norm_bwd_apply_kernel<T>), bgrid, dim3(256), 0,
                                            (hipStream_t)stream, (const T*)dy, (const T*)y, (const T*)x, (const T*)r, k1, k2,
                                            (T*)dx, (T*)dr, HW, C, units, relu, scale1, shift1, scale2, shift2));
  AST_CHECK_LAUNCH();
  return 0;
}

extern "C" int ast_norm_bwd_apply(const void* dy, const void* y, const void* x, const void* r, const float* k1,
                                  const float* k2, void* dx, void* dr, int N, int HW, int C, int relu, int dtype,
                                  void* stream) {
  return ast_norm_bwd_apply_pre(dy, y, x, r, k1, k2, dx, dr, N, HW, C, relu, dtype, nullptr, nullptr, nullptr, nullptr, stream);
}

extern "C" int ast_bn_apply_fwd(const void* x, const void* r, void* y, const float* tab1, int rows1, long count1, const float* tab2,
                               const float* gamma1, const float* beta1, float* running_mean, float* running_var, int64_t* num_batches_tracked,
                               float eps1, const float* gamma2, const float* beta2, float eps2, float* out1, float* out2, int N, int HW, int C,
                               int Creal, int relu, int dtype, void* stream) {
  if (!x || !y || !tab1 || !gamma1 || !beta1 || !out1 || rows1 < 1 || count1 < 1 || N < 1 || HW < 1 || C < 8 || (C & 7) || C > 2048 || Creal > C)
    AST_FAIL("ast_bn_apply_fwd: bad args (rows %d count %ld N %d HW %d C %d)", rows1, count1, N, HW, C);
  if (r && (!tab2 || !gamma2 || !beta2 || !out2)) AST_FAIL("ast_bn_apply_fwd: the second (InstanceNorm) input needs its table, gamma / beta and out2");
  if ((long)rows1 * C > 65536) AST_FAIL("ast_bn_apply_fwd: statistics table too large for the in-kernel reduction (rows %d x C %d)", rows1, C);
  const int nparts = std::max(1, std::min(rows1, 256 / std::min(C, 256)));
  const size_t lds = sizeof(float) * (size_t)(4 * C + 2 * C * nparts);
  const dim3 grid(std::max(1, std::min<int>((int)(((size_t)HW * (C >> 3) + 255) / 256), std::max(1, elem_blocks() / N))), N);
  AST_DISPATCH_T(dtype, hipLaunchKernelGGL((bn_apply_fwd_kernel<T>), grid, dim3(256), lds, (hipStream_t)stream, (const T*)x, (const T*)r, (T*)y, tab1,
                                            rows1, (float)count1, tab2, gamma1, beta1, running_mean, running_var, num_batches_tracked, eps1, gamma2,
                                            beta2, eps2, out1, out2, N, HW, C, Creal, relu));
  AST_CHECK_LAUNCH();
  return 0;
}

extern "C" int ast_bn_apply_bwd(const void* dy, const void* x, const void* r, void* dx, void* dr, const float* tab3, int rows, long count,
                               const float* gamma1, const float* mean1, const float* rstd1, float* dgamma1, float* dbeta1,
                               const float* gamma2, const float* mean2, const float* rstd2, float* dgamma2, float* dbeta2,
                               const float* scale1, const float* shift1, const float* scale2, const float* shift2, int N, int HW, int C,
                               int Creal, int relu, int dtype, void* stream) {
  if (!dy || !x || !dx || !tab3 || !gamma1 || !mean1 || !rstd1 || rows < 1 || count < 1 || N < 1 || HW < 1 || C < 8 || (C & 7) || C > 2048 || Creal > C)
    AST_FAIL("ast_bn_apply_bwd: bad args (rows %d count %ld N %d HW %d C %d)", rows, count, N, HW, C);
  if (dr && (!r || !gamma2 || !mean2 || !rstd2 || rows != N)) AST_FAIL("ast_bn_apply_bwd: the instance branch needs r, gamma2 / mean2 / rstd2 and a per-image table (rows == N)");
  if (relu && (!scale1 || !shift1 || (r && (!scale2 || !shift2)))) AST_FAIL("ast_bn_apply_bwd: the ReLU mask is recomputed from the pre-activation: scale / shift required");
  if ((long)rows * C > 65536) AST_FAIL("ast_bn_apply_bwd: statistics table too large for the in-kernel reduction (rows %d x C %d)", rows, C);
  const int nparts = std::max(1, std::min(rows, 256 / std::min(C, 256)));
  const size_t lds = sizeof(float) * (size_t)(6 * C + 2 * C * nparts);
  const dim3 grid(std::max(1, std::min<int>((int)(((size_t)HW * (C >> 3) + 255) / 256), std::max(1, elem_blocks() / N))), N);
  AST_DISPATCH_T(dtype, hipLaunchKernelGGL((bn_apply_bwd_kernel<T>), grid, dim3(256), lds, (hipStream_t)stream, (const T*)dy, (const T*)x, (const T*)r,
                                            (T*)dx, (T*)dr, tab3, rows, (float)count, gamma1, mean1, rstd1, dgamma1, dbeta1, gamma2, mean2, rstd2,
                                            dgamma2, dbeta2, scale1, shift1, scale2, shift2, N, HW, C, Creal, relu));
  AST_CHECK_LAUNCH();
  return 0;
}

extern "C" int ast_layernorm_fwd(const void* x, const float* gamma, const float* beta, void* y, float* mean, float* rstd,
                                 int rows, int D, float eps, int dtype, void* stream) {
  if (dtype != AST_F32) AST_FAIL("ast_layernorm_fwd: f32 only (token tensors are kept in f32)");
  if (!x || !gamma || !beta || !y || !mean || !rstd || rows <= 0 || D <= 0) AST_FAIL("ast_layernorm_fwd: bad args");
  hipLaunchKernelGGL(layernorm_fwd_kernel, dim3((rows + 3) / 4), dim3(256), 0, (hipStream_t)stream, (const float*)x, gamma,
                     beta, (float*)y, mean, rstd, rows, D, eps);
  AST_CHECK_LAUNCH();
  return 0;
}

extern "C" int ast_layernorm_bwd(const void* dy, const void* x, const float* gamma, const float* mean, const float* rstd,
                                 void* dx, float* dgamma, float* dbeta, int rows, int D, int dtype, void* stream) {
  if (dtype != AST_F32) AST_FAIL("ast_layernorm_bwd: f32 only");
  if (!dy || !x || !gamma || !mean || !rstd || !dx || rows <= 0 || D <= 0) AST_FAIL("ast_layernorm_bwd: bad args");
  hipLaunchKernelGGL(layernorm_bwd_kernel<false>, dim3((rows + 3) / 4), dim3(256), 0, (hipStream_t)stream, (const float*)dy,
                     (const float*)x, gamma, mean, rstd, (float*)dx, dgamma, dbeta, rows, D);
  AST_CHECK_LAUNCH();
  return 0;
}

extern "C" int ast_add_drop_ln_fwd(const float* x, const float* sub, float* mask, float* s_out, const float* gamma, const float* beta,
                                   float* y, float* mean, float* rstd, int rows, int D, float eps, float p, uint64_t seed,
                                   const int64_t* d_offset, void* stream) {
  if (!sub || !s_out || rows <= 0 || D <= 0 || p < 0.f || p >= 1.f) AST_FAIL("ast_add_drop_ln_fwd: bad args");
  if (p > 0.f && !mask) AST_FAIL("ast_add_drop_ln_fwd: dropout needs a mask buffer");
  if (gamma && (!beta || !y || !mean || !rstd)) AST_FAIL("ast_add_drop_ln_fwd: LayerNorm outputs missing");
  const bool al = ((((uintptr_t)x) | ((uintptr_t)sub) | ((uintptr_t)mask) | ((uintptr_t)s_out) | ((uintptr_t)gamma) | ((uintptr_t)beta) |
                    ((uintptr_t)y)) & 15) == 0;
  if (D == 256 && al)
    hipLaunchKernelGGL(add_drop_ln_fwd256_kernel, dim3((rows + 3) / 4), dim3(256), 0, (hipStream_t)stream, x, sub, mask, s_out, gamma,
                       beta, y, mean, rstd, rows, eps, p, seed, d_offset);
  else
    hipLaunchKernelGGL(add_drop_ln_fwd_kernel, dim3((rows + 3) / 4), dim3(256), 0, (hipStream_t)stream, x, sub, mask, s_out, gamma, beta,
                       y, mean, rstd, rows, D, eps, p, seed, d_offset);
  AST_CHECK_LAUNCH();
  return 0;
}

extern "C" int ast_add_drop_ln_bwd(const float* dy, const float* ds_ext, const float* s, const float* gamma, const float* mean,
                                   const float* rstd, const float* mask, float* dx, float* dsub, float* dgamma, float* dbeta, int rows,
                                   int D, void* stream) {
  if ((!dy && !ds_ext) || !dsub || rows <= 0 || D <= 0) AST_FAIL("ast_add_drop_ln_bwd: bad args");
  if (dy && (!s || !gamma || !mean || !rstd)) AST_FAIL("ast_add_drop_ln_bwd: LayerNorm state missing");
  const bool al = ((((uintptr_t)dy) | ((uintptr_t)ds_ext) | ((uintptr_t)s) | ((uintptr_t)gamma) | ((uintptr_t)mask) | ((uintptr_t)dx) |
                    ((uintptr_t)dsub)) & 15) == 0;
  if (D == 256 && al)
    hipLaunchKernelGGL(add_drop_ln_bwd256_kernel, dim3((rows + 3) / 4), dim3(256), 0, (hipStream_t)stream, dy, ds_ext, s, gamma, mean, rstd,
                       mask, dx, dsub, dgamma, dbeta, rows);
  else
    hipLaunchKernelGGL(add_drop_ln_bwd_kernel<false>, dim3((rows + 3) / 4), dim3(256), 0, (hipStream_t)stream, dy, ds_ext, s, gamma, mean, rstd,
                       mask, dx, dsub, dgamma, dbeta, rows, D);
  AST_CHECK_LAUNCH();
  return 0;
}

extern "C" int ast_ordered_sum(const float* parts, int64_t n, int nslots, int batches, float* out, int accumulate, void* stream);

extern "C" int ast_chan_stats_det(const void* x, float* sums, int N, int HW, int C, int dtype, float* ws, int nslots, void* stream) {
  if (!x || !sums || !ws || N <= 0 || HW <= 0 || C <= 0 || (C & 7) || C > 2048 || nslots < 1 || nslots > AST_DET_MAX_SLOTS)
    AST_FAIL("ast_chan_stats_det: bad args N=%d HW=%d C=%d slots=%d", N, HW, C, nslots);
  hipStream_t s = (hipStream_t)stream;
  const int ppb = (HW + nslots - 1) / nslots;
  const float* nf = nullptr;
  AST_DISPATCH_T(dtype, hipLaunchKernelGGL((chan_reduce_kernel<T, 0, true>), dim3(nslots, N), dim3(256), 0, s, (const T*)x, (const T*)nullptr,
                                            (const T*)nullptr, (const T*)nullptr, ws, HW, C, ppb, 0, nf, nf, nf, nf));
  AST_CHECK_LAUNCH();
  return ast_ordered_sum(ws, (int64_t)C * 2, nslots, N, sums, 0, stream);
}

extern "C" int ast_norm_bwd_sums_det(const void* dy, const void* y, const void* x, const void* r, float* sums3, int N, int HW, int C, int relu,
                                     int dtype, const float* scale1, const float* shift1, const float* scale2, const float* shift2, float* ws,
                                     int nslots, void* stream) {
  if (!dy || !x || !sums3 || !ws || (relu && !y && !scale1) || (C & 7) || C <= 0 || C > 2048 || N <= 0 || HW <= 0 || nslots < 1 ||
      nslots > AST_DET_MAX_SLOTS)
    AST_FAIL("ast_norm_bwd_sums_det: bad args");
  if (scale1 && (!shift1 || (r && (!scale2 || !shift2)))) AST_FAIL("ast_norm_bwd_sums_det: incomplete pre-activation coefficients");
  hipStream_t s = (hipStream_t)stream;
  const int ppb = (HW + nslots - 1) / nslots;
  AST_DISPATCH_T(dtype, hipLaunchKernelGGL((chan_reduce_kernel<T, 1, true>), dim3(nslots, N), dim3(256), 0, s, (const T*)dy, (const T*)y,
                                            (const T*)x, (const T*)r, ws, HW, C, ppb, relu, scale1, shift1, scale2, shift2));
  AST_CHECK_LAUNCH();
  return ast_ordered_sum(ws, (int64_t)C * 3, nslots, N, sums3, 0, stream);
}

extern "C" int ast_layernorm_bwd_det(const void* dy, const void* x, const float* gamma, const float* mean, const float* rstd, void* dx,
                                     float* dgamma, float* dbeta, int rows, int D, int dtype, float* ws, void* stream) {
  if (dtype != AST_F32) AST_FAIL("ast_layernorm_bwd_det: f32 only");
  if (!dy || !x || !gamma || !mean || !rstd || !dx || !ws || rows <= 0 || rows > AST_DET_MAX_SLOTS || D <= 0)
    AST_FAIL("ast_layernorm_bwd_det: bad args (1..%d rows)", AST_DET_MAX_SLOTS);
  hipLaunchKernelGGL(layernorm_bwd_kernel<true>, dim3((rows + 3) / 4), dim3(256), 0, (hipStream_t)stream, (const float*)dy,
                     (const float*)x, gamma, mean, rstd, (float*)dx, dgamma ? ws : nullptr, dbeta ? ws + (size_t)rows * D : nullptr, rows, D);
  AST_CHECK_LAUNCH();
  if (dgamma) if (int rc = ast_ordered_sum(ws, D, rows, 1, dgamma, 1, stream)) return rc;
  if (dbeta) if (int rc = ast_ordered_sum(ws + (size_t)rows * D, D, rows, 1, dbeta, 1, stream)) return rc;
  return 0;
}

extern "C" int ast_add_drop_ln_bwd_det(const float* dy, const float* ds_ext, const float* s, const float* gamma, const float* mean,
                                       const float* rstd, const float* mask, float* dx, float* dsub, float* dgamma, float* dbeta, int rows,
                                       int D, float* ws, void* stream) {
  if ((!dy && !ds_ext) || !dsub || rows <= 0 || rows > AST_DET_MAX_SLOTS || D <= 0) AST_FAIL("ast_add_drop_ln_bwd_det: bad args");
  if (dy && (!s || !gamma || !mean || !rstd)) AST_FAIL("ast_add_drop_ln_bwd_det: LayerNorm state missing");
  const bool red = dy && (dgamma || dbeta);
  if (red && !ws) AST_FAIL("ast_add_drop_ln_bwd_det: the gamma / beta gradients need 2 * rows * D floats of ws");
  hipLaunchKernelGGL(add_drop_ln_bwd_kernel<true>, dim3((rows + 3) / 4), dim3(256), 0, (hipStream_t)stream, dy, ds_ext, s, gamma, mean, rstd,
                     mask, dx, dsub, red && dgamma ? ws : nullptr, red && dbeta ? ws + (size_t)rows * D : nullptr, rows, D);
  AST_CHECK_LAUNCH();
  if (red && dgamma) if (int rc = ast_ordered_sum(ws, D, rows, 1, dgamma, 1, stream)) return rc;
  if (red && dbeta) if (int rc = ast_ordered_sum(ws + (size_t)rows * D, D, rows, 1, dbeta, 1, stream)) return rc;
  return 0;
}
```

### audio-style-transfer_amd/csrc/skinny.hip

```cpp
#include "ast_common.h"
#include "../../include/ast_hip.h"

namespace {

template <int NW, int RT>
__device__ __forceinline__ f32x4 sum_partials(const f32x4 (&part)[NW][RT][64], int t, int lane) {
  f32x4 r = part[0][t][lane];
#pragma unroll
  for (int q = 1; q < NW; ++q) { const f32x4 p = part[q][t][lane]; r[0] += p[0]; r[1] += p[1]; r[2] += p[2]; r[3] += p[3]; }
  return r;
}

template <int RT, int NS, int NW>
__global__ __launch_bounds__(64 * NW) void skinny_gemm_kernel(const float* __restrict__ x, const float* __restrict__ w,
                                                           const float* __restrict__ bias, float* __restrict__ y, int M, int N,
                                                           int K, int ldx, int ldw, int ldy, int relu,
                                                           const float* __restrict__ mul_mask, float* __restrict__ drop_mask,
                                                           float p, uint64_t seed, const int64_t* __restrict__ d_offset) {
  __shared__ f32x4 part[NW][RT][64];
  const int lane = threadIdx.x & 63, wave = threadIdx.x >> 6;
  const int i = lane & 15, g = lane >> 4;
  const int n0 = blockIdx.x * 16, m0 = blockIdx.y * 16 * RT;
  constexpr int kslice = NS * 16;
  const int kb = wave * kslice;
  const bool nv = n0 + i < N;
  const float* wr = w + (size_t)(nv ? n0 + i : 0) * ldw;
  const float* xr[RT];
  bool mv[RT];
  f32x4 acc[RT];
#pragma unroll
  for (int t = 0; t < RT; ++t) {
    const int m = m0 + 16 * t + i;
    mv[t] = m < M;
    xr[t] = x + (size_t)(mv[t] ? m : 0) * ldx;
    acc[t] = f32x4{0.f, 0.f, 0.f, 0.f};
  }
  float bq[4] = {0.f, 0.f, 0.f, 0.f};
  if (bias) {
#pragma unroll
    for (int q = 0; q < 4; ++q) { const int n = n0 + 4 * g + q; bq[q] = bias[n < N ? n : 0]; }
  }
  f32x4 wl[NS], xl[RT][NS];
#pragma unroll
  for (int s = 0; s < NS; ++s) {
    const int k = kb + s * 16 + 4 * g;
    const int kc = k < K ? k : 0;
    wl[s] = *reinterpret_cast<const f32x4*>(wr + kc);
#pragma unroll
    for (int t = 0; t < RT; ++t) xl[t][s] = *reinterpret_cast<const f32x4*>(xr[t] + kc);
  }
  __builtin_amdgcn_sched_barrier(0);
#pragma unroll
  for (int s = 0; s < NS; ++s) {
    const bool kv = kb + s * 16 + 4 * g < K;
    const f32x4 z = {0.f, 0.f, 0.f, 0.f};
    const f32x4 a = (kv && nv) ? wl[s] : z;
#pragma unroll
    for (int t = 0; t < RT; ++t) {
      const f32x4 b = (kv && mv[t]) ? xl[t][s] : z;
#pragma unroll
      for (int e = 0; e < 4; ++e) acc[t] = __builtin_amdgcn_mfma_f32_16x16x4f32(a[e], b[e], acc[t], 0, 0, 0);
    }
  }
#pragma unroll
  for (int t = 0; t < RT; ++t) part[wave][t][lane] = acc[t];
  __syncthreads();
  if (wave >= RT) return;
  const int m = m0 + 16 * wave + i, nb = n0 + 4 * g;
  if (m >= M) return;
  const f32x4 r = sum_partials(part, wave, lane);
  const uint64_t base = drop_mask ? mix64(seed ^ mix64((uint64_t)(d_offset ? *d_offset : 0))) : 0;
  const float keep = 1.f / (1.f - p);
#pragma unroll
  for (int q = 0; q < 4; ++q) {
    const int n = nb + q;
    if (n < N) {
      const size_t o = (size_t)m * ldy + n;
      float v = r[q] + bq[q];
      if (relu) v = fmaxf(v, 0.f);
      if (drop_mask) {
        const float km = dropout_keep(base, o, p, keep);
        drop_mask[o] = (relu && v <= 0.f) ? 0.f : km;
        v *= km;
      }
      if (mul_mask) v *= mul_mask[o];
      y[o] = v;
    }
  }
}

template <int NS, int NW>
__global__ __launch_bounds__(64 * NW) void bign_gemm_len_kernel(const float* __restrict__ x, const float* __restrict__ w,
                                                             const float* __restrict__ bias, float* __restrict__ y, int M, int N,
                                                             int K, int ldw, int ldy, int S, const int32_t* __restrict__ n_valid) {
  constexpr int RT = 4;
  __shared__ f32x4 part[NW][RT][64];
  const int lane = threadIdx.x & 63, wave = threadIdx.x >> 6;
  const int i = lane & 15, g = lane >> 4;
  const int n0 = blockIdx.y * 16, m0 = blockIdx.x * 16 * RT;
  const int kb = wave * NS * 16;
  const bool nv = n0 + i < N;
  const float* wr = w + (size_t)(nv ? n0 + i : 0) * ldw;
  const float* xr[RT];
  bool mv[RT], live[RT];
  bool any_live = false;
  f32x4 acc[RT];
#pragma unroll
  for (int t = 0; t < RT; ++t) {
    const int m = m0 + 16 * t + i;
    mv[t] = m < M;
    if (mv[t] && n_valid) {
      const int b = m / S, nb = n_valid[b];
      mv[t] = m - b * S < (nb < 1 ? 1 : nb > S ? S : nb);
    }
    live[t] = __any(mv[t]);
    any_live = any_live || live[t];
    xr[t] = x + (size_t)(mv[t] ? m : 0) * K;
    acc[t] = f32x4{0.f, 0.f, 0.f, 0.f};
  }
  if (!any_live) {
    const int m = m0 + 16 * wave + i;
    if (wave < RT && m < M) {
#pragma unroll
      for (int q = 0; q < 4; ++q)
        if (n0 + 4 * g + q < N) y[(size_t)m * ldy + n0 + 4 * g + q] = 0.f;
    }
    return;
  }
  float bq[4] = {0.f, 0.f, 0.f, 0.f};
  if (bias) {
#pragma unroll
    for (int q = 0; q < 4; ++q) { const int n = n0 + 4 * g + q; bq[q] = bias[n < N ? n : 0]; }
  }
  f32x4 wl[NS], xl[RT][NS];
#pragma unroll
  for (int s = 0; s < NS; ++s) {
    const int k = kb + s * 16 + 4 * g;
    const int kc = k < K ? k : 0;
    wl[s] = *reinterpret_cast<const f32x4*>(wr + kc);
  }
#pragma unroll
  for (int t = 0; t < RT; ++t) {
#pragma unroll
    for (int s = 0; s < NS; ++s) xl[t][s] = f32x4{0.f, 0.f, 0.f, 0.f};
    if (!live[t]) continue;
#pragma unroll
    for (int s = 0; s < NS; ++s) {
      const int k = kb + s * 16 + 4 * g;
      xl[t][s] = *reinterpret_cast<const f32x4*>(xr[t] + (k < K ? k : 0));
    }
  }
  __builtin_amdgcn_sched_barrier(0);
#pragma unroll
  for (int s = 0; s < NS; ++s) {
    const bool kv = kb + s * 16 + 4 * g < K;
    const f32x4 z = {0.f, 0.f, 0.f, 0.f};
    const f32x4 a = (kv && nv) ? wl[s] : z;
#pragma unroll
    for (int t = 0; t < RT; ++t) {
      if (!live[t]) continue;
      const f32x4 b = (kv && mv[t]) ? xl[t][s] : z;
#pragma unroll
      for (int e = 0; e < 4; ++e) acc[t] = __builtin_amdgcn_mfma_f32_16x16x4f32(a[e], b[e], acc[t], 0, 0, 0);
    }
  }
#pragma unroll
  for (int t = 0; t < RT; ++t) part[wave][t][lane] = acc[t];
  __syncthreads();
// ... 165 lines not shown
  if (wave >= RT) return;
  const int m = m0 + 16 * wave + i, nb = n0 + 4 * g;
  if (m >= M) return;
  const f32x4 r = sum_partials(part, wave, lane);
#pragma unroll
  for (int q = 0; q < 4; ++q) {
    const int n = nb + q;
    if (n >= N) continue;
    const float v = r[q] + ((bias && blockIdx.z == 0) ? bias[n] : 0.f);
    if constexpr (DET) y[((size_t)blockIdx.z * M + m) * N + n] = v;
    else unsafeAtomicAdd(y + (size_t)m * ldy + n, v);
  }
}

template <int RT, bool DET>
__global__ __launch_bounds__(256) void bign_dgrad_kernel(const float* __restrict__ dy, const float* __restrict__ w,
                                                          float* __restrict__ dx, int M, int N, int K, int lddy) {
  const int lane = threadIdx.x & 63, wave = threadIdx.x >> 6;
  const int i = lane & 15, g = lane >> 4;
  const int nb0 = blockIdx.x * 512, m0 = blockIdx.y * 16 * RT;
  const int kt0 = wave * 4;
  const float* dr[RT];
  bool mv[RT];
  f32x4 acc[RT][4];
#pragma unroll
  for (int u = 0; u < RT; ++u) {
    const int m = m0 + 16 * u + i;
    mv[u] = m < M;
    dr[u] = dy + (size_t)(mv[u] ? m : 0) * lddy;
#pragma unroll
    for (int t = 0; t < 4; ++t) acc[u][t] = f32x4{0.f, 0.f, 0.f, 0.f};
  }
#pragma unroll 1
  for (int sb = 0; sb < 128; sb += 8) {
    float a[8][4], b[RT][8];
#pragma unroll
    for (int s = 0; s < 8; ++s) {
      const int n = nb0 + (sb + s) * 4 + g;
      const int nc = n < N ? n : 0;
#pragma unroll
      for (int u = 0; u < RT; ++u) b[u][s] = dr[u][nc];
      const float* wrow = w + (size_t)nc * K;
#pragma unroll
      for (int t = 0; t < 4; ++t) {
        const int k = (kt0 + t) * 16 + i;
        a[s][t] = wrow[k < K ? k : 0];
      }
    }
    __builtin_amdgcn_sched_barrier(0);
#pragma unroll
    for (int s = 0; s < 8; ++s) {
      const bool nvv = nb0 + (sb + s) * 4 + g < N;
#pragma unroll
      for (int t = 0; t < 4; ++t) {
        const float aq = (nvv && (kt0 + t) * 16 + i < K) ? a[s][t] : 0.f;
#pragma unroll
        for (int u = 0; u < RT; ++u) {
          const float bq = (nvv && mv[u]) ? b[u][s] : 0.f;
          acc[u][t] = __builtin_amdgcn_mfma_f32_16x16x4f32(aq, bq, acc[u][t], 0, 0, 0);
        }
      }
    }
  }
#pragma unroll
  for (int u = 0; u < RT; ++u) {
    const int m = m0 + 16 * u + i;
    if (m >= M) continue;
#pragma unroll
    for (int t = 0; t < 4; ++t)
#pragma unroll
      for (int r = 0; r < 4; ++r) {
        const int k = (kt0 + t) * 16 + 4 * g + r;
        if (k >= K) continue;
        if constexpr (DET) dx[((size_t)blockIdx.x * M + m) * K + k] = acc[u][t][r];
        else unsafeAtomicAdd(dx + (size_t)m * K + k, acc[u][t][r]);
      }
  }
}

template <int RT> constexpr int rows_lo() { return RT == 1 ? 1 : 65; }
template <int RT> constexpr int rows_hi() { return RT == 1 ? 64 : AST_WIDE_MAX_ROWS; }
template <int RT> constexpr bool rows_ok(int M) { return M >= rows_lo<RT>() && M <= rows_hi<RT>(); }

template <int RT>
int skinny_gemm_launch(const char* name, const float* x, const float* w, const float* bias, float* y, int M, int N, int K, int ldw,
                       int ldy, int relu, const float* mul_mask, float* drop_mask, float p, uint64_t seed, const int64_t* d_offset,
                       void* stream) {
  if (!x || !w || !y || !rows_ok<RT>(M) || N < 1 || K < 4 || (K & 3) || (ldw & 3) || (RT > 1 && (ldw < K || ldy < N)))
    AST_FAIL("%s: bad args M=%d (%d..%d) N=%d K=%d ldw=%d ldy=%d", name, M, rows_lo<RT>(), rows_hi<RT>(), N, K, ldw, ldy);
  if ((((uintptr_t)x) | ((uintptr_t)w)) & 15) AST_FAIL("%s: operands must be 16-byte aligned", name);
  if (drop_mask && (p <= 0.f || p >= 1.f)) AST_FAIL("%s: dropout epilogue needs 0 < p < 1", name);
  const int steps = (K + 63) / 64;
  if (steps > 16) AST_FAIL("%s: K=%d too large for the token path (<= 1024)", name, K);
  dim3 grid((N + 15) / 16, (M + 16 * RT - 1) / (16 * RT));
#define AST_SK(NS_, NW_) hipLaunchKernelGGL((skinny_gemm_kernel<RT, NS_, NW_>), grid, dim3(64 * NW_), 0, (hipStream_t)stream, x, w, bias, y, \
                                            M, N, K, K, ldw, ldy, relu, mul_mask, drop_mask, p, seed, d_offset)
  if (steps <= 2) AST_SK(2, 4);
  else if (steps <= 4) AST_SK(4, 4);
  else if (steps <= 8) AST_SK(8, 4);
  else AST_SK(8, 8);
#undef AST_SK
  AST_CHECK_LAUNCH();
  return 0;
}

int bign_gemm_len_launch(const char* name, const float* x, const float* w, const float* bias, float* y, int M, int N, int K, int ldw,
                         int ldy, int S, const int32_t* n_valid, void* stream) {
  if (!x || !w || !y || M < 1 || M > AST_BIGN_MAX_ROWS || S < 1 || M % S || N < 1 || K < 4 || (K & 3) || (ldw & 3) || ldw < K || ldy < N)
    AST_FAIL("%s: bad args M=%d (1..%d) S=%d (M %% S == 0) N=%d K=%d ldw=%d ldy=%d", name, M, AST_BIGN_MAX_ROWS, S, N, K, ldw, ldy);
  if ((((uintptr_t)x) | ((uintptr_t)w)) & 15) AST_FAIL("%s: operands must be 16-byte aligned", name);
  if ((((uintptr_t)y) | ((uintptr_t)bias) | ((uintptr_t)n_valid)) & 3) AST_FAIL("%s: y, bias and n_valid must be 4-byte aligned", name);
  const int steps = (K + 63) / 64;
  if (steps > 16) AST_FAIL("%s: K=%d too large for the token path (<= 1024)", name, K);
  if ((N + 15) / 16 > 65535) AST_FAIL("%s: N=%d too large (<= %d)", name, N, 65535 * 16);
  dim3 grid((M + 63) / 64, (N + 15) / 16);
#define AST_BL(NS_, NW_) hipLaunchKernelGGL((bign_gemm_len_kernel<NS_, NW_>), grid, dim3(64 * NW_), 0, (hipStream_t)stream, x, w, bias, y, \
                                            M, N, K, ldw, ldy, S, n_valid)
  if (steps <= 2) AST_BL(2, 4);
  else if (steps <= 4) AST_BL(4, 4);
  else if (steps <= 8) AST_BL(8, 4);
  else AST_BL(8, 8);
#undef AST_BL
  AST_CHECK_LAUNCH();
  return 0;
}

template <int RT>
int linear_wgrad_launch(const char* name, const float* dy, const float* x, float* dW, float* db, int M, int N, int K, int lddy, int ldw,
                        void* stream) {
  if (!dy || !x || !dW || !rows_ok<RT>(M) || N < 1 || K < 1 || (RT > 1 && (lddy < N || ldw < K)))
    AST_FAIL("%s: bad args M=%d (%d..%d token rows) N=%d K=%d lddy=%d ldw=%d", name, M, rows_lo<RT>(), rows_hi<RT>(), N, K, lddy, ldw);
  dim3 grid((K + 63) / 64, (N + 63) / 64);
  if (RT > 1 && grid.y > 65535) AST_FAIL("%s: N=%d too large", name, N);
  hipStream_t s = (hipStream_t)stream;
  if (RT > 1) hipLaunchKernelGGL(linear_wgrad_rows_kernel, grid, dim3(256), 0, s, dy, x, dW, db, M, N, K, lddy, ldw);
  else if (M <= 16) hipLaunchKernelGGL(linear_wgrad_kernel<4>, grid, dim3(256), 0, s, dy, x, dW, db, M, N, K, lddy, ldw);
  else if (M <= 32) hipLaunchKernelGGL(linear_wgrad_kernel<8>, grid, dim3(256), 0, s, dy, x, dW, db, M, N, K, lddy, ldw);
  else hipLaunchKernelGGL(linear_wgrad_kernel<16>, grid, dim3(256), 0, s, dy, x, dW, db, M, N, K, lddy, ldw);
  AST_CHECK_LAUNCH();
  return 0;
}

template <int RT, bool DET>
int bigk_gemm_launch(const char* name, const float* x, const float* w, const float* bias, float* y, int M, int N, int K, int ldy, float* ws,
                     long ws_floats, void* stream) {
  if (!x || !w || !y || (DET && !ws) || !rows_ok<RT>(M) || N < 1 || K < 2 || (K & 1) || (RT > 1 && ldy < N))
    AST_FAIL("%s: bad args M=%d (%d..%d) N=%d K=%d (K must be even) ldy=%d", name, M, rows_lo<RT>(), rows_hi<RT>(), N, K, ldy);
  if ((((uintptr_t)x) | ((uintptr_t)w)) & 7) AST_FAIL("%s: operands must be 8-byte aligned", name);
  const int nz = (K + 1023) / 1024;
  if ((RT > 1 || DET) && nz > (RT > 1 ? 65535 : AST_DET_MAX_SLOTS)) AST_FAIL("%s: K=%d too large", name, K);
  if (DET && ws_floats < (long)nz * M * N) AST_FAIL("%s: ws needs %ld floats", name, (long)nz * M * N);
  dim3 grid((N + 15) / 16, (M + 16 * RT - 1) / (16 * RT), nz);
  if (!DET) AST_HIP(hipMemsetAsync(y, 0, sizeof(float) * (size_t)M * ldy, (hipStream_t)stream));
  hipLaunchKernelGGL((bigk_gemm_kernel<RT, DET>), grid, dim3(256), 0, (hipStream_t)stream, x, w, bias, DET ? ws : y, M, N, K, ldy);
  AST_CHECK_LAUNCH();
  return DET ? ast_ordered_sum(ws, (int64_t)M * N, nz, 1, y, 0, stream) : 0;
}

template <int RT, bool DET>
int bign_dgrad_launch(const char* name, const float* dy, const float* w, float* dx, int M, int N, int K, int lddy, float* ws, long ws_floats,
                      void* stream) {
  if (!dy || !w || !dx || (DET && !ws) || !rows_ok<RT>(M) || N < 1 || K < 1 || K > 256 || (RT > 1 && lddy < N))
    AST_FAIL("%s: bad args M=%d (%d..%d) N=%d K=%d (K <= 256) lddy=%d", name, M, rows_lo<RT>(), rows_hi<RT>(), N, K, lddy);
  const int nx = (N + 511) / 512;
  if (DET && (nx > AST_DET_MAX_SLOTS || ws_floats < (long)nx * M * K)) AST_FAIL("%s: ws needs %ld floats", name, (long)nx * M * K);
  dim3 grid(nx, (M + 16 * RT - 1) / (16 * RT));
  if (!DET) AST_HIP(hipMemsetAsync(dx, 0, sizeof(float) * (size_t)M * K, (hipStream_t)stream));
  hipLaunchKernelGGL((bign_dgrad_kernel<RT, DET>), grid, dim3(256), 0, (hipStream_t)stream, dy, w, DET ? ws : dx, M, N, K, lddy);
  AST_CHECK_LAUNCH();
  return DET ? ast_ordered_sum(ws, (int64_t)M * K, nx, 1, dx, 0, stream) : 0;
}
}

extern "C" int ast_linear_wgrad_batched_host(const void* host_table, int count, int max_tiles, void* stream) {
  if (!host_table || count <= 0 || max_tiles <= 0) AST_FAIL("ast_linear_wgrad_batched_host: bad args");
  const LinWg* recs = (const LinWg*)host_table;
  for (int c0 = 0; c0 < count; c0 += LINWG_MAX) {
    const int n = std::min(LINWG_MAX, count - c0);
    LinWgArgs args;
// ... 20 lines not shown

extern "C" int ast_skinny_gemm(const float* x, const float* w, const float* bias, float* y, int M, int N, int K, int ldw, int ldy,
                               int relu, void* stream) {
  return skinny_gemm_launch<1>("ast_skinny_gemm", x, w, bias, y, M, N, K, ldw, ldy, relu, nullptr, nullptr, 0.f, 0, nullptr, stream);
}

extern "C" int ast_linear_wgrad(const float* dy, const float* x, float* dW, float* db, int M, int N, int K, int lddy, int ldw,
                                void* stream) {
  return linear_wgrad_launch<1>("ast_linear_wgrad", dy, x, dW, db, M, N, K, lddy, ldw, stream);
}

extern "C" int ast_bigk_gemm(const float* x, const float* w, const float* bias, float* y, int M, int N, int K, int ldy, void* stream) {
  return bigk_gemm_launch<1, false>("ast_bigk_gemm", x, w, bias, y, M, N, K, ldy, nullptr, 0, stream);
}

extern "C" long ast_bigk_gemm_det_ws_floats(int M, int N, int K) {
  if (!rows_ok<1>(M) || N < 1 || K < 2) return -1;
  return (long)((K + 1023) / 1024) * M * N;
}

extern "C" int ast_bigk_gemm_det(const float* x, const float* w, const float* bias, float* y, int M, int N, int K, float* ws, long ws_floats,
                                 void* stream) {
  return bigk_gemm_launch<1, true>("ast_bigk_gemm_det", x, w, bias, y, M, N, K, N, ws, ws_floats, stream);
}

extern "C" int ast_bign_dgrad(const float* dy, const float* w, float* dx, int M, int N, int K, int lddy, void* stream) {
  return bign_dgrad_launch<1, false>("ast_bign_dgrad", dy, w, dx, M, N, K, lddy, nullptr, 0, stream);
}

extern "C" long ast_bign_dgrad_det_ws_floats(int M, int N, int K) {
  if (!rows_ok<1>(M) || N < 1 || K < 1 || K > 256) return -1;
  return (long)((N + 511) / 512) * M * K;
}

extern "C" int ast_bign_dgrad_det(const float* dy, const float* w, float* dx, int M, int N, int K, int lddy, float* ws, long ws_floats,
                                  void* stream) {
  return bign_dgrad_launch<1, true>("ast_bign_dgrad_det", dy, w, dx, M, N, K, lddy, ws, ws_floats, stream);
}

extern "C" int ast_skinny_gemm_wide_ex(const float* x, const float* w, const float* bias, float* y, int M, int N, int K, int ldw, int ldy,
                                       int relu, const float* mul_mask, float* drop_mask, float p, uint64_t seed, const int64_t* d_offset,
                                       void* stream) {
  return skinny_gemm_launch<4>("ast_skinny_gemm_wide", x, w, bias, y, M, N, K, ldw, ldy, relu, mul_mask, drop_mask, p, seed, d_offset, stream);
}

extern "C" int ast_skinny_gemm_wide(const float* x, const float* w, const float* bias, float* y, int M, int N, int K, int ldw, int ldy,
                                    int relu, void* stream) {
  return skinny_gemm_launch<4>("ast_skinny_gemm_wide", x, w, bias, y, M, N, K, ldw, ldy, relu, nullptr, nullptr, 0.f, 0, nullptr, stream);
}

extern "C" int ast_linear_wgrad_wide(const float* dy, const float* x, float* dW, float* db, int M, int N, int K, int lddy, int ldw,
                                     void* stream) {
  return linear_wgrad_launch<4>("ast_linear_wgrad_wide", dy, x, dW, db, M, N, K, lddy, ldw, stream);
}

extern "C" int ast_bigk_gemm_wide(const float* x, const float* w, const float* bias, float* y, int M, int N, int K, int ldy, void* stream) {
  return bigk_gemm_launch<4, false>("ast_bigk_gemm_wide", x, w, bias, y, M, N, K, ldy, nullptr, 0, stream);
}

extern "C" long ast_bigk_gemm_wide_det_ws_floats(int M, int N, int K) {
  if (!rows_ok<4>(M) || N < 1 || K < 2 || (K & 1) || (K + 1023) / 1024 > 65535) return -1;
  return (long)((K + 1023) / 1024) * M * N;
}

extern "C" int ast_bigk_gemm_wide_det(const float* x, const float* w, const float* bias, float* y, int M, int N, int K, float* ws,
                                      long ws_floats, void* stream) {
  return bigk_gemm_launch<4, true>("ast_bigk_gemm_wide_det", x, w, bias, y, M, N, K, N, ws, ws_floats, stream);
}

extern "C" int ast_bign_dgrad_wide(const float* dy, const float* w, float* dx, int M, int N, int K, int lddy, void* stream) {
  return bign_dgrad_launch<4, false>("ast_bign_dgrad_wide", dy, w, dx, M, N, K, lddy, nullptr, 0, stream);
}

extern "C" long ast_bign_dgrad_wide_det_ws_floats(int M, int N, int K) {
  if (!rows_ok<4>(M) || N < 1 || K < 1 || K > 256 || (N + 511) / 512 > AST_DET_MAX_SLOTS) return -1;
  return (long)((N + 511) / 512) * M * K;
}

extern "C" int ast_bign_dgrad_wide_det(const float* dy, const float* w, float* dx, int M, int N, int K, int lddy, float* ws,
                                       long ws_floats, void* stream) {
  return bign_dgrad_launch<4, true>("ast_bign_dgrad_wide_det", dy, w, dx, M, N, K, lddy, ws, ws_floats, stream);
}

extern "C" int ast_bign_gemm_len(const float* x, const float* w, const float* bias, float* y, int M, int N, int K, int ldw, int ldy, int S,
                                 const int32_t* n_valid, void* stream) {
  return bign_gemm_len_launch("ast_bign_gemm_len", x, w, bias, y, M, N, K, ldw, ldy, S, n_valid, stream);
}
```

### include/ast_hip.h

```cpp
#ifndef AST_HIP_H
#define AST_HIP_H
#include <stddef.h>
#include <stdint.h>
#ifdef __cplusplus
extern "C" {
#endif

#define AST_DTYPE_F32 0
#define AST_DTYPE_BF16 1
#define AST_MAX_TAPS 9

int ast_version(void);
const char* ast_last_error(void);

typedef struct ast_gather_t {
  int32_t N, Hs, Ws, Cs;
  int32_t Hm, Wm;
  int32_t sh, sw, oh, ow;
  int32_t Hd, Wd, Cd;
  int32_t dsh, dsw, doh, dow;
  int32_t ntaps, wtaps;
  int32_t tap[AST_MAX_TAPS];
} ast_gather_t;

// ... 230 lines not shown
long ast_mfcc_distance_ws_floats(int B, int n_gen, int n_ref, int hop);
int ast_mfcc_distance_len(const float* generated, int n_gen, const float* reference, int n_ref, int B, const int32_t* len_gen,
                          const int32_t* len_ref, int n_mfcc, int hop, int pad_mode, const int32_t* mel_table, float* ws, long ws_floats,
                          float* out, void* stream);

int ast_chroma_run_frames(void);
int ast_pitch_band(int n_fft, int* k_lo, int* k_hi);
int ast_tuning_debug_words(void);
long ast_tuning_ws_floats(int B, int n, int n_fft);
int ast_tuning_len(const float* waves, int B, int n, const int32_t* n_samples, const int32_t* n_cut, int cut_max, int n_fft, int hop,
                   int pad_mode, float* ws, long ws_floats, float* tuning, int32_t* debug, void* stream);
int ast_chroma_len(const float* waves, int B, int n, const int32_t* n_samples, const int32_t* n_cut, int cut_max, int n_fft, int hop,
                   int pad_mode, const float* tuning, float* out, void* stream);
long ast_chroma_distance_ws_floats(int B, int n_orig, int n_gen);
int ast_chroma_distance_len(const float* original, int n_orig, const float* generated, int n_gen, int B, const int32_t* len_orig,
                            const int32_t* len_gen, int pad_mode, float* ws, long ws_floats, float* out, void* stream);
long ast_chroma_similarity_ws_floats(int B, int n_gen, int n_orig);
int ast_chroma_similarity_len(const float* generated, int n_gen, const float* original, int n_orig, int B, const int32_t* len_gen,
                              const int32_t* len_orig, int pad_mode, float* ws, long ws_floats, float* out, void* stream);
int ast_pitch_mean_len(const float* waves, int B, int n, const int32_t* n_samples, const int32_t* n_cut, int cut_max, int pad_mode,
                       float* out, void* stream);
long ast_pitch_correlation_ws_floats(int B, int n_orig, int n_gen);
int ast_pitch_correlation_len(const float* original, int n_orig, const float* generated, int n_gen, int B, const int32_t* len_orig,
                              const int32_t* len_gen, int pad_mode, float* ws, long ws_floats, float* out, void* stream);

int ast_onset_tile_frames(void);
int ast_recurrence_chunk_frames(void);
long ast_onset_strength_ws_floats(int B, int n);
int ast_onset_strength_len(const float* waves, int B, int n, const int32_t* n_samples, int pad_mode, const int32_t* mel_table, float* ws,
                           long ws_floats, float* out, void* stream);
long ast_onset_detect_ws_floats(int B, int n);
int ast_onset_detect_len(const float* waves, int B, int n, const int32_t* n_samples, int pad_mode, const int32_t* mel_table, float* ws,
                         long ws_floats, int32_t* mask, void* stream);
long ast_onset_accuracy_ws_floats(int B, int n_orig, int n_gen);
int ast_onset_accuracy_len(const float* original, int n_orig, const float* generated, int n_gen, int B, const int32_t* len_orig,
                           const int32_t* len_gen, int pad_mode, const int32_t* mel_table, float* ws, long ws_floats, float* out,
                           void* stream);
long ast_recurrence_ws_floats(int B, int n);
int ast_recurrence_len(const float* waves, int B, int n, const int32_t* n_samples, int pad_mode, const int32_t* mel_table, float* ws,
                       long ws_floats, int32_t* R, float* dist2, void* stream);
long ast_self_similarity_distance_ws_floats(int B, int n_a, int n_b);
int ast_self_similarity_distance_len(const float* a, int n_a, const float* b, int n_b, int B, const int32_t* len_a, const int32_t* len_b,
                                     int pad_mode, const int32_t* mel_table, float* ws, long ws_floats, float* out, void* stream);

#define AST_DET_MAX_SLOTS 65536
#define AST_IGEMM_DETERMINISTIC 4096
int ast_ordered_sum(const float* parts, int64_t n, int nslots, int batches, float* out, int accumulate, void* stream);
long ast_igemm_ws_floats_det(const ast_gather_t* g, int dtype);
int ast_sumsq_det(const float* x, int64_t n, float* out, float* ws, int nslots, void* stream);
int ast_colsum_acc_det(const void* x, int64_t rows, int C, int Creal, float* out, int dtype, float* ws, int nslots, void* stream);
int ast_chan_stats_det(const void* x, float* sums, int N, int HW, int C, int dtype, float* ws, int nslots, void* stream);
int ast_norm_bwd_sums_det(const void* dy, const void* y, const void* x, const void* r, float* sums3, int N, int HW, int C, int relu,
                          int dtype, const float* scale1, const float* shift1, const float* scale2, const float* shift2, float* ws,
                          int nslots, void* stream);
int ast_layernorm_bwd_det(const void* dy, const void* x, const float* gamma, const float* mean, const float* rstd, void* dx,
                          float* dgamma, float* dbeta, int rows, int D, int dtype, float* ws, void* stream);
int ast_add_drop_ln_bwd_det(const float* dy, const float* ds_ext, const float* s, const float* gamma, const float* mean,
                            const float* rstd, const float* mask, float* dx, float* dsub, float* dgamma, float* dbeta, int rows,
                            int D, float* ws, void* stream);
int ast_recon_loss_total_det(const float* out, const float* tgt, int64_t tgt_ld, int B, int S, int T, int Fq, const float* coef5,
                             const float* inv5, float* ws, long ws_floats, float* res11, float* grad, void* stream);
long ast_bigk_gemm_det_ws_floats(int M, int N, int K);
int ast_bigk_gemm_det(const float* x, const float* w, const float* bias, float* y, int M, int N, int K, float* ws, long ws_floats, void* stream);
long ast_bign_dgrad_det_ws_floats(int M, int N, int K);
int ast_bign_dgrad_det(const float* dy, const float* w, float* dx, int M, int N, int K, int lddy, float* ws, long ws_floats, void* stream);
int ast_weight_grads_flush_det(const ast_weight_desc_t* descs, const void* tiles, int ntiles, float* ws, long ws_floats, void* stream);

#define AST_WIDE_MAX_ROWS 1024
int ast_skinny_gemm_wide(const float* x, const float* w, const float* bias, float* y, int M, int N, int K, int ldw, int ldy, int relu,
                         void* stream);
int ast_skinny_gemm_wide_ex(const float* x, const float* w, const float* bias, float* y, int M, int N, int K, int ldw, int ldy,
                            int relu, const float* mul_mask, float* drop_mask, float p, uint64_t seed, const int64_t* d_offset,
                            void* stream);
int ast_linear_wgrad_wide(const float* dy, const float* x, float* dW, float* db, int M, int N, int K, int lddy, int ldw, void* stream);
int ast_bigk_gemm_wide(const float* x, const float* w, const float* bias, float* y, int M, int N, int K, int ldy, void* stream);
long ast_bigk_gemm_wide_det_ws_floats(int M, int N, int K);
int ast_bigk_gemm_wide_det(const float* x, const float* w, const float* bias, float* y, int M, int N, int K, float* ws, long ws_floats,
                           void* stream);
int ast_bign_dgrad_wide(const float* dy, const float* w, float* dx, int M, int N, int K, int lddy, void* stream);
long ast_bign_dgrad_wide_det_ws_floats(int M, int N, int K);
int ast_bign_dgrad_wide_det(const float* dy, const float* w, float* dx, int M, int N, int K, int lddy, float* ws, long ws_floats,
                            void* stream);

#define AST_BIGN_MAX_ROWS 4096
int ast_bign_gemm_len(const float* x, const float* w, const float* bias, float* y, int M, int N, int K, int ldw, int ldy, int S,
                      const int32_t* n_valid , void* stream);

enum { AST_TOK_GEMM = 1, AST_TOK_ATTN_FWD = 2, AST_TOK_ATTN_BWD = 3, AST_TOK_ADLN_FWD = 4, AST_TOK_ADLN_BWD = 5 };
enum { AST_TOK_RELU = 1, AST_TOK_NO_BARRIER = 2, AST_TOK_CAUSAL = 4 };
typedef struct {
  int32_t type, flags;
  int32_t i[8];
  float p, eps;
  uint64_t seed;
  const float* in[7];
  float* out[5];
} ast_tok_op_t;
int ast_tok_max_ops(void);
int ast_tok_program(const ast_tok_op_t* ops, int nops, int G, int xcd, void* sync, int* status, const int64_t* d_offset,
                    void* stream);

int ast_frame_rms_tile_frames(void);
int ast_mfcc_mean_chunk_frames(void);
long ast_frame_rms_ws_floats(int B, int n);
int ast_frame_rms_len(const float* waves, int B, int n, const int32_t* n_samples, float threshold, int pad_mode, float* ws,
                      long ws_floats, float* rms, int32_t* n_frames, int32_t* silent, float* silence_ratio, float* level,
                      double* sumsq, void* stream);
int ast_window_sound_len(const float* waves, int B, int n, const int32_t* n_samples, int win, float threshold_db, int32_t* mask,
                         float* sound_ratio, void* stream);
long ast_mfcc_mean_ws_floats(int B, int n, int hop);
int ast_mfcc_mean_len(const float* waves, int B, int n, const int32_t* n_samples, int n_mfcc, int hop, int pad_mode,
                      const int32_t* mel_table, float* ws, long ws_floats, float* out, void* stream);
int ast_gain_rows_len(const float* waves, int B, int n, const int32_t* n_samples, const double* sumsq, double target_rms, float* out,
                      void* stream);

int ast_state_digest(const void* const* ptrs, const long long* nbytes, int n, unsigned long long* out, void* stream);

#ifdef __cplusplus
}
#endif
#endif
```

Measured before the change: 5338 audio-seconds/sec.

## Fuse transformer layers into single autograd functions with accumulating backward kernels

Adds whole-layer autograd Functions for the encoder layer and the full decoder stack. They chain the existing fused ops directly, so per-op autograd nodes and Python dispatch disappear. Backward passes now fold residual-gradient additions into the skinny GEMM and layernorm backward kernels through new accumulate (_acc) variants, which drops separate add kernels and temporary tensors. The change makes the backward path harder to read, and the new path is skipped in deterministic mode under the auto setting.

After: 5384 audio-seconds/sec (median of 6 runs). Within noise of the previous version (+0.9%).

```diff
diff --git a/audio-style-transfer_amd/ast_amd/_lib.py b/audio-style-transfer_amd/ast_amd/_lib.py
--- a/audio-style-transfer_amd/ast_amd/_lib.py
+++ b/audio-style-transfer_amd/ast_amd/_lib.py
@@ -133,6 +133,12 @@
     "ast_bign_dgrad_wide": ([vp, vp, vp, i32, i32, i32, i32, vp], i32),
     "ast_bign_dgrad_wide_det_ws_floats": ([i32, i32, i32], C.c_long),
     "ast_bign_dgrad_wide_det": ([vp, vp, vp, i32, i32, i32, i32, vp, C.c_long, vp], i32),
+    "ast_skinny_gemm_acc": ([vp, vp, vp, vp, i32, i32, i32, i32, i32, i32, vp, vp, f32, C.c_uint64, vp, vp, i32, vp], i32),
+    "ast_skinny_gemm_wide_acc": ([vp, vp, vp, vp, i32, i32, i32, i32, i32, i32, vp, vp, f32, C.c_uint64, vp, vp, i32, vp], i32),
+    "ast_layernorm_bwd_acc": ([vp, vp, vp, vp, vp, vp, vp, vp, i32, i32, i32, vp, vp], i32),
+    "ast_layernorm_bwd_det_acc": ([vp, vp, vp, vp, vp, vp, vp, vp, i32, i32, i32, vp, vp, vp], i32),
+    "ast_add_drop_ln_bwd_acc": ([vp, vp, vp, vp, vp, vp, vp, vp, vp, vp, vp, i32, i32, vp, vp, vp], i32),
+    "ast_add_drop_ln_bwd_det_acc": ([vp, vp, vp, vp, vp, vp, vp, vp, vp, vp, vp, i32, i32, vp, vp, vp, vp], i32),
     "ast_tok_max_ops": ([], i32),
     "ast_tok_program": ([vp, i32, i32, i32, vp, vp, vp, vp], i32),
     "ast_attn_fwd_len": ([vp, vp, vp, vp, vp, i32, i32, i32, i32, i32, i32, i32, i32, i32, vp, i32, vp], i32),
diff --git a/audio-style-transfer_amd/ast_amd/config.py b/audio-style-transfer_amd/ast_amd/config.py
--- a/audio-style-transfer_amd/ast_amd/config.py
+++ b/audio-style-transfer_amd/ast_amd/config.py
@@ -13,6 +13,13 @@
 import os as _os
 fused_tokens = _os.environ.get("AST_FUSED_TOKENS", "1") != "0"
 tok_programs = int(_os.environ.get("AST_TOK_PROGRAMS", "0"))
+
+token_layers = _os.environ.get("AST_TOKEN_LAYERS", "auto")
+
+
+def token_layers_enabled():
+    return token_layers not in ("0", "") and (token_layers != "auto" or not deterministic)
+
 
 fused_bn_stats = _os.environ.get("AST_FUSED_BN_STATS", "1") != "0"
 
diff --git a/audio-style-transfer_amd/ast_amd/decoder_trunk.py b/audio-style-transfer_amd/ast_amd/decoder_trunk.py
--- a/audio-style-transfer_amd/ast_amd/decoder_trunk.py
+++ b/audio-style-transfer_amd/ast_amd/decoder_trunk.py
@@ -66,6 +66,10 @@
         if (self.token_programs and lengths is None and config.tok_programs > 0
                 and tokprog.decoder_stack_ok(tgt, memory, self._layers)):
             return tokprog.decoder_stack(tgt, memory, self._layers, self.training)
+        if lengths is None:
+            out = L.decoder_stack(self._layers, tgt, memory, self.training)
+            if out is not None:
+                return out
         for lyr in self._layers:
             tgt = lyr(tgt, memory, self.training, lengths)
         return tgt
diff --git a/audio-style-transfer_amd/ast_amd/layers.py b/audio-style-transfer_amd/ast_amd/layers.py
--- a/audio-style-transfer_amd/ast_amd/layers.py
+++ b/audio-style-transfer_amd/ast_amd/layers.py
@@ -459,6 +459,115 @@
         return linear(o, self.out).view(B, Lq, d)
 
 
+def _run(fn, *args):
+    c = ops.OpCtx()
+    return c, fn.forward(c, *args)
+
+
+def _lin_fwd(x2d, pw, relu=False):
+    return _run(ops.LinearFn, x2d, pw.weight, pw, relu)
+
+
+def _attn_fwd(q, kv, B, H, Lq, Lk, dh, k_off, v_off, causal, p):
+    return _run(ops.AttnCoreFn, q, kv, B, H, Lq, Lk, dh, k_off, v_off, causal, p)
+
+
+def _layer_pws_ok(pws, rows):
+    return all(ops._skinny_ok(pw, rows) for pw in pws)
+
+
+def token_layers_on(*tensors):
+    return (config.fused_tokens and config.token_layers_enabled() and torch.is_grad_enabled()
+            and all(t.dtype == torch.float32 and t.dim() == 3 for t in tensors))
+
+
+class EncoderLayerFn(torch.autograd.Function):
+
+    @staticmethod
+    def forward(ctx, x, anchor, lyr, training):
+        l, at = lyr.l, lyr.attn
+        B, L, d = x.shape
+        rows, dh = B * L, d // at.h
+        drop = lambda p: float(p) if training else 0.0
+        c = {}
+        c["qkv"], qkv = _lin_fwd(x.reshape(rows, d), at.qkv)
+        c["att"], o = _attn_fwd(qkv, qkv, B, at.h, L, L, dh, d, 2 * d, False, drop(l.self_attn.dropout))
+        c["out"], a = _lin_fwd(o, at.out)
+        c["n1"], (_, x1) = _run(ops.AddDropLNFn, x, a.view(B, L, d), l.norm1, drop(l.dropout1.p))
+        c["ffn"], h = _run(ops.FFNFn, x1.reshape(rows, d), lyr.ff1.weight, lyr.ff2.weight, lyr.ff1, lyr.ff2, drop(l.dropout.p))
+        c["n2"], (_, y) = _run(ops.AddDropLNFn, x1, h.view(B, L, d), l.norm2, drop(l.dropout2.p))
+        ctx.ops = c
+        return y
+
+    @staticmethod
+    def backward(ctx, dy):
+        c = ctx.ops
+        dx1, dh = ops.AddDropLNFn.backward(c["n2"], None, dy)[:2]
+        dx1 = ops.FFNFn.backward(c["ffn"], dh.reshape(-1, dh.shape[-1]), addend=dx1)[0]
+        dx, da = ops.AddDropLNFn.backward(c["n1"], None, dx1.view(dy.shape))[:2]
+        do = ops.LinearFn.backward(c["out"], da.reshape(-1, da.shape[-1]))[0]
+        dqkv = ops.AttnCoreFn.backward(c["att"], do)[0]
+        dx = ops.LinearFn.backward(c["qkv"], dqkv, addend=dx)[0]
+        return dx.view(dy.shape), None, None, None
+
+
+class DecoderStackFn(torch.autograd.Function):
+
+    @staticmethod
+    def forward(ctx, x, memory, anchor, lyrs, training):
+        B, L, d = x.shape
+        Lm = memory.shape[1]
+        rows = B * L
+        drop = lambda p: float(p) if training else 0.0
+        mem2 = memory.reshape(B * Lm, d)
+        states = []
+        for lyr in lyrs:
+            l, sa, ca = lyr.l, lyr.sa, lyr.ca
+            c = {}
+            c["ln1"], h = _run(ops.LayerNormFn, x, l.norm1.weight, l.norm1.bias, l.norm1.eps)
+            c["qkv"], qkv = _lin_fwd(h.reshape(rows, d), sa.qkv)
+            c["sa"], o = _attn_fwd(qkv, qkv, B, sa.h, L, L, d // sa.h, d, 2 * d, True, drop(l.self_attn.dropout))
+            c["so"], a = _lin_fwd(o, sa.out)
+            c["n2"], (x, h) = _run(ops.AddDropLNFn, x, a.view(B, L, d), l.norm2, drop(l.dropout1.p))
+            c["q"], q = _lin_fwd(h.reshape(rows, d), ca.q)
+            c["kv"], kv = _lin_fwd(mem2, ca.kv)
+            c["ca"], o = _attn_fwd(q, kv, B, ca.h, L, Lm, d // ca.h, 0, d, False, drop(l.multihead_attn.dropout))
+            c["co"], a = _lin_fwd(o, ca.out)
+            c["n3"], (x, h) = _run(ops.AddDropLNFn, x, a.view(B, L, d), l.norm3, drop(l.dropout2.p))
+            c["ffn"], f = _run(ops.FFNFn, h.reshape(rows, d), lyr.ff1.weight, lyr.ff2.weight, lyr.ff1, lyr.ff2, drop(l.dropout.p))
+            c["n4"], x = _run(ops.AddDropLNFn, x, f.view(B, L, d), None, drop(l.dropout3.p))
+            states.append(c)
+        ctx.ops, ctx.mem_shape = states, memory.shape
+        return x
+
+    @staticmethod
+    def backward(ctx, dx):
+        shape, d = dx.shape, dx.shape[-1]
+        flat = lambda t: t.reshape(-1, t.shape[-1])
+        dmem = None
+        for c in reversed(ctx.ops):
+            dx, df = ops.AddDropLNFn.backward(c["n4"], dx, None)[:2]
+            dh = ops.FFNFn.backward(c["ffn"], flat(df))[0]
+            dx, da = ops.AddDropLNFn.backward(c["n3"], dx, dh.view(shape))[:2]
+            do = ops.LinearFn.backward(c["co"], flat(da))[0]
+            dq, dkv = ops.AttnCoreFn.backward(c["ca"], do)[:2]
+            dmem = ops.LinearFn.backward(c["kv"], dkv, addend=dmem)[0]
+            dh = ops.LinearFn.backward(c["q"], dq)[0]
+            dx, da = ops.AddDropLNFn.backward(c["n2"], dx, dh.view(shape))[:2]
+            do = ops.LinearFn.backward(c["so"], flat(da))[0]
+            dqkv = ops.AttnCoreFn.backward(c["sa"], do)[0]
+            dh = ops.LinearFn.backward(c["qkv"], dqkv)[0]
+            dx = ops.LayerNormFn.backward(c["ln1"], dh.view(shape), addend=dx)[0]
+        return dx, dmem.view(ctx.mem_shape), None, None, None
+
+
+def decoder_stack(lyrs, x, memory, training):
+    B, L, d = x.shape
+    if not (lyrs and token_layers_on(x, memory) and all(lyr.layer_fn_ok(B * L, B * memory.shape[1]) for lyr in lyrs)):
+        return None
+    return DecoderStackFn.apply(x, memory, lyrs[0].ff1.weight, lyrs, bool(training))
+
+
 class EncoderLayer:
 
     def __init__(self, bank, layer: nn.TransformerEncoderLayer):
@@ -467,10 +576,15 @@
         self.ff1 = bank.add(layer.linear1.weight, "linear", tok_dtype, bias=layer.linear1.bias)
         self.ff2 = bank.add(layer.linear2.weight, "linear", tok_dtype, bias=layer.linear2.bias)
 
+    def layer_fn_ok(self, rows):
+        return _layer_pws_ok((self.attn.qkv, self.attn.out, self.ff1, self.ff2), rows)
+
     def __call__(self, x, training, lengths=None):
         l, p = self.l, self.l.dropout.p
         B, L, d = x.shape
         km = None if lengths is None else (lengths, L)
+        if lengths is None and token_layers_on(x) and self.layer_fn_ok(B * L):
+            return EncoderLayerFn.apply(x, self.ff1.weight, self, bool(training))
         if not config.fused_tokens:
             x = layer_norm(x + ops.dropout(self.attn(x, None, training, l.self_attn.dropout, key_mask=km), l.dropout1.p, training),
                            l.norm1)
@@ -492,10 +606,18 @@
         self.ff1 = bank.add(layer.linear1.weight, "linear", tok_dtype, bias=layer.linear1.bias)
         self.ff2 = bank.add(layer.linear2.weight, "linear", tok_dtype, bias=layer.linear2.bias)
 
+    def layer_fn_ok(self, rows, mrows):
+        return (_layer_pws_ok((self.sa.qkv, self.sa.out, self.ca.q, self.ca.out, self.ff1, self.ff2), rows)
+                and _layer_pws_ok((self.ca.kv,), mrows))
+
     def __call__(self, x, memory, training, lengths=None):
         l = self.l
         B, L, d = x.shape
         km = None if lengths is None else (lengths, memory.shape[1] // 2)
+        if lengths is None:
+            y = decoder_stack([self], x, memory, training)
+            if y is not None:
+                return y
         if not config.fused_tokens:
             h = layer_norm(x, l.norm1)
             x = x + ops.dropout(self.sa(h, None, training, l.self_attn.dropout, causal=True), l.dropout1.p, training)
diff --git a/audio-style-transfer_amd/ast_amd/ops.py b/audio-style-transfer_amd/ast_amd/ops.py
--- a/audio-style-transfer_amd/ast_amd/ops.py
+++ b/audio-style-transfer_amd/ast_amd/ops.py
@@ -419,6 +419,35 @@
     check(getattr(lib(), name)(*args, stream()), name)
 
 
+def _token_gemm(who, rows, *args, ex=None, addend=None):
+    if addend is None:
+        _token_call(who, "skinny_gemm", rows, "_ex" if ex else "", *args, *(ex or ()))
+        return
+    assert addend.dim() == 2 and addend.shape[0] == rows and addend.stride(1) == 1 and addend.dtype == torch.float32, addend.shape
+    _token_call(who, "skinny_gemm", rows, "_acc", *args, *(ex or (None, None, 0.0, 0, None)), ptr(addend), addend.stride(0))
+
+
+def _rows2d(t, rows):
+    t = t.reshape(rows, -1)
+    return t if t.stride(1) == 1 else t.contiguous()
+
+
+class OpCtx:
+    needs_input_grad = (True,) * 16
+
+    def __init__(self):
+        self.saved_tensors = ()
+
+    def save_for_backward(self, *tensors):
+        self.saved_tensors = tensors
+
+    def set_materialize_grads(self, flag):
+        pass
+
+    def mark_non_differentiable(self, *tensors):
+        pass
+
+
 def _token_rows_ok(rows):
     return rows <= SKINNY_MAX_ROWS or (config.deterministic and rows <= WIDE_MAX_ROWS)
 
@@ -446,11 +475,12 @@
         return y
 
     @staticmethod
-    def backward(ctx, dy):
+    def backward(ctx, dy, addend=None):
         x, y = ctx.saved_tensors
         pw = ctx.pw
         dy = dy.contiguous()
         rows = x.shape[0]
+        assert addend is None or ctx.skinny
         if ctx.relu:
             dz = torch.empty_like(dy)
             check(lib().ast_relu_bwd(ptr(dy), ptr(y), ptr(dz), dy.numel(), dcode(dy.dtype), stream()), "ast_relu_bwd")
@@ -465,7 +495,8 @@
                 _token_call("LinearFn", "linear_wgrad", rows, "", ptr(dy), ptr(x), gw.data_ptr() + 4 * pw.w_off, gb, rows, pw.Co, pw.Ci, pw.Cop, pw.s_co)
             if ctx.needs_input_grad[0]:
                 dx = torch.empty_like(x)
-                _token_call("LinearFn", "skinny_gemm", rows, "", ptr(dy), ptr(pw.wb), None, ptr(dx), rows, pw.Ci, pw.Cop, pw.Cop, pw.Cip, 0)
+                _token_gemm("LinearFn", rows, ptr(dy), ptr(pw.wb), None, ptr(dx), rows, pw.Ci, pw.Cop, pw.Cop, pw.Cip, 0,
+                            addend=None if addend is None else _rows2d(addend, rows))
             return dx, None, None, None
         if config.deterministic:
             raise RuntimeError(f"LinearFn: the non-skinny weight gradient (> {WIDE_MAX_ROWS} token rows, spectral norm, unpadded channels "
@@ -572,7 +603,7 @@
         return y
 
     @staticmethod
-    def backward(ctx, dy):
+    def backward(ctx, dy, addend=None):
         x, h, mask = ctx.saved_tensors
         pw1, pw2 = ctx.pw1, ctx.pw2
         dy = dy.contiguous()
@@ -591,7 +622,8 @@
         dx = None
         if ctx.needs_input_grad[0]:
             dx = torch.empty_like(x)
-            _token_call("FFNFn", "skinny_gemm", rows, "", ptr(dh), ptr(pw1.wb), None, ptr(dx), rows, pw1.Ci, pw1.Cop, pw1.Cop, pw1.Cip, 0)
+            _token_gemm("FFNFn", rows, ptr(dh), ptr(pw1.wb), None, ptr(dx), rows, pw1.Ci, pw1.Cop, pw1.Cop, pw1.Cip, 0,
+                        addend=None if addend is None else _rows2d(addend, rows))
         return dx, None, None, None, None, None
 
 
@@ -869,19 +901,23 @@
         return y.view(shape)
 
     @staticmethod
-    def backward(ctx, dy):
+    def backward(ctx, dy, addend=None):
         x2, mean, rstd = ctx.saved_tensors
         rows, D = x2.shape
         dy2 = dy.contiguous().view(rows, D)
         dx = torch.empty_like(x2)
+        add2 = None if addend is None else addend.contiguous().view(rows, D)
+        acc, tail = ("", ()) if add2 is None else ("_acc", (ptr(add2),))
         if config.deterministic:
-            check(lib().ast_layernorm_bwd_det(ptr(dy2), ptr(x2), ptr(ctx.gamma), ptr(mean), ptr(rstd), ptr(dx), ptr(acc_grad(ctx.gamma)),
-                                              ptr(acc_grad(ctx.beta)), rows, D, dcode(x2.dtype), ptr(det_ws(2 * rows * D, dx.device)),
-                                              stream()), "ast_layernorm_bwd_det")
+            name = "ast_layernorm_bwd_det" + acc
+            check(getattr(lib(), name)(ptr(dy2), ptr(x2), ptr(ctx.gamma), ptr(mean), ptr(rstd), ptr(dx), ptr(acc_grad(ctx.gamma)),
+                                       ptr(acc_grad(ctx.beta)), rows, D, dcode(x2.dtype), ptr(det_ws(2 * rows * D, dx.device)),
+                                       *tail, stream()), name)
             return dx.view(ctx.shape), None, None, None
-        check(lib().ast_layernorm_bwd(ptr(dy2), ptr(x2), ptr(ctx.gamma), ptr(mean), ptr(rstd), ptr(dx),
-                                      ptr(acc_grad(ctx.gamma)), ptr(acc_grad(ctx.beta)), rows, D, dcode(x2.dtype),
-                                      stream()), "ast_layernorm_bwd")
+        name = "ast_layernorm_bwd" + acc
+        check(getattr(lib(), name)(ptr(dy2), ptr(x2), ptr(ctx.gamma), ptr(mean), ptr(rstd), ptr(dx),
+                                   ptr(acc_grad(ctx.gamma)), ptr(acc_grad(ctx.beta)), rows, D, dcode(x2.dtype),
+                                   *tail, stream()), name)
         return dx.view(ctx.shape), None, None, None
 
 
diff --git a/audio-style-transfer_amd/csrc/ast_common.h b/audio-style-transfer_amd/csrc/ast_common.h
--- a/audio-style-transfer_amd/csrc/ast_common.h
+++ b/audio-style-transfer_amd/csrc/ast_common.h
@@ -116,6 +116,11 @@
   return v;
 }
 
+__device__ __forceinline__ float add_rn(float a, float b) {
+  asm("" : "+v"(a));
+  return a + b;
+}
+
 __device__ __forceinline__ uint64_t mix64(uint64_t z) {
   z += 0x9E3779B97F4A7C15ull; z = (z ^ (z >> 30)) * 0xBF58476D1CE4E5B9ull; z = (z ^ (z >> 27)) * 0x94D049BB133111EBull; return z ^ (z >> 31);
 }
diff --git a/audio-style-transfer_amd/csrc/norm.hip b/audio-style-transfer_amd/csrc/norm.hip
--- a/audio-style-transfer_amd/csrc/norm.hip
+++ b/audio-style-transfer_amd/csrc/norm.hip
@@ -524,11 +524,11 @@
   if (lane == 0) { mean[row] = m; rstd[row] = r; }
 }
 
-template <bool DET = false>
+template <bool DET = false, bool ACC = false>
 __global__ void layernorm_bwd_kernel(const float* __restrict__ dy, const float* __restrict__ x,
                                      const float* __restrict__ gamma, const float* __restrict__ mean,
                                      const float* __restrict__ rstd, float* __restrict__ dx, float* dgamma, float* dbeta,
-                                     int rows, int D) {
+                                     int rows, int D, const float* __restrict__ dx_add = nullptr) {
   const int row = blockIdx.x * (blockDim.x >> 6) + (threadIdx.x >> 6), lane = threadIdx.x & 63;
   if (row >= rows) return;
   const float m = mean[row], r = rstd[row];
@@ -542,7 +542,8 @@
   a = wave_sum(a) / D; b = wave_sum(b) / D;
   for (int i = lane; i < D; i += 64) {
     const float xh = (xr[i] - m) * r, g = dr[i] * gamma[i];
-    dx[(size_t)row * D + i] = r * (g - a - xh * b);
+    if constexpr (ACC) dx[(size_t)row * D + i] = add_rn(r * (g - a - xh * b), dx_add[(size_t)row * D + i]);
+    else dx[(size_t)row * D + i] = r * (g - a - xh * b);
     if constexpr (DET) {
       if (dgamma) dgamma[(size_t)row * D + i] = dr[i] * xh;
       if (dbeta) dbeta[(size_t)row * D + i] = dr[i];
@@ -580,11 +581,12 @@
   if (lane == 0) { mean[row] = m; rstd[row] = r; }
 }
 
-template <bool DET = false>
+template <bool DET = false, bool ACC = false>
 __global__ void add_drop_ln_bwd_kernel(const float* __restrict__ dy, const float* __restrict__ ds_ext, const float* __restrict__ s,
                                        const float* __restrict__ gamma, const float* __restrict__ mean, const float* __restrict__ rstd,
                                        const float* __restrict__ mask, float* __restrict__ dx, float* __restrict__ dsub,
-                                       float* dgamma, float* dbeta, int rows, int D) {
+                                       float* dgamma, float* dbeta, int rows, int D, const float* __restrict__ dx_add = nullptr,
+                                       const float* __restrict__ dsub_add = nullptr) {
   const int row = blockIdx.x * (blockDim.x >> 6) + (threadIdx.x >> 6), lane = threadIdx.x & 63;
   if (row >= rows) return;
   const size_t o = (size_t)row * D;
@@ -610,8 +612,14 @@
         if (dbeta) unsafeAtomicAdd(dbeta + i, dy[o + i]);
       }
     }
-    if (dx) dx[o + i] = d;
-    dsub[o + i] = mask ? d * mask[o + i] : d;
+    if constexpr (ACC) {
+      if (dx) dx[o + i] = dx_add ? add_rn(d, dx_add[o + i]) : d;
+      const float ds = mask ? d * mask[o + i] : d;
+      dsub[o + i] = dsub_add ? add_rn(ds, dsub_add[o + i]) : ds;
+    } else {
+      if (dx) dx[o + i] = d;
+      dsub[o + i] = mask ? d * mask[o + i] : d;
+    }
   }
 }
 
@@ -657,11 +665,14 @@
   if (lane == 0) { mean[row] = m; rstd[row] = r; }
 }
 
+template <bool ACC = false>
 __global__ __launch_bounds__(256) void add_drop_ln_bwd256_kernel(const float* __restrict__ dy, const float* __restrict__ ds_ext,
                                                                  const float* __restrict__ s, const float* __restrict__ gamma,
                                                                  const float* __restrict__ mean, const float* __restrict__ rstd,
                                                                  const float* __restrict__ mask, float* __restrict__ dx,
-                                                                 float* __restrict__ dsub, float* dgamma, float* dbeta, int rows) {
+                                                                 float* __restrict__ dsub, float* dgamma, float* dbeta, int rows,
+                                                                 const float* __restrict__ dx_add = nullptr,
+                                                                 const float* __restrict__ dsub_add = nullptr) {
   constexpr int D = 256;
   __shared__ float red[2][4][D];
   const int wave = threadIdx.x >> 6, lane = threadIdx.x & 63;
@@ -675,6 +686,11 @@
   const f32x4 e4 = ds_ext ? *reinterpret_cast<const f32x4*>(ds_ext + o) : z;
   const f32x4 k4 = mask ? *reinterpret_cast<const f32x4*>(mask + o) : f32x4{1.f, 1.f, 1.f, 1.f};
   const float m = dy ? mean[valid ? row : 0] : 0.f, r = dy ? rstd[valid ? row : 0] : 0.f;
+  f32x4 xa4 = z, sa4 = z;
+  if constexpr (ACC) {
+    if (dx && dx_add) xa4 = *reinterpret_cast<const f32x4*>(dx_add + o);
+    if (dsub_add) sa4 = *reinterpret_cast<const f32x4*>(dsub_add + o);
+  }
   __builtin_amdgcn_sched_barrier(0);
   f32x4 d4 = e4, xh4 = z;
   if (dy) {
@@ -686,10 +702,20 @@
     for (int e = 0; e < 4; ++e) d4[e] += r * (dy4[e] * g4[e] - a - xh4[e] * b);
   }
   if (valid) {
-    if (dx) *reinterpret_cast<f32x4*>(dx + o) = d4;
     f32x4 ds4;
 #pragma unroll
     for (int e = 0; e < 4; ++e) ds4[e] = d4[e] * k4[e];
+    if constexpr (ACC) {
+      f32x4 dx4 = d4;
+#pragma unroll
+      for (int e = 0; e < 4; ++e) {
+        if (dx_add) dx4[e] = add_rn(d4[e], xa4[e]);
+        if (dsub_add) ds4[e] = add_rn(ds4[e], sa4[e]);
+      }
+      if (dx) *reinterpret_cast<f32x4*>(dx + o) = dx4;
+    } else {
+      if (dx) *reinterpret_cast<f32x4*>(dx + o) = d4;
+    }
     *reinterpret_cast<f32x4*>(dsub + o) = ds4;
   }
   if (dy && (dgamma || dbeta)) {
@@ -865,14 +891,25 @@
   return 0;
 }
 
+template <bool ACC>
+static int layernorm_bwd_launch(const char* name, const void* dy, const void* x, const float* gamma, const float* mean, const float* rstd,
+                                void* dx, float* dgamma, float* dbeta, int rows, int D, int dtype, const float* dx_add, void* stream) {
+  if (dtype != AST_F32) AST_FAIL("%s: f32 only", name);
+  if (!dy || !x || !gamma || !mean || !rstd || !dx || rows <= 0 || D <= 0 || (ACC && (!dx_add || dx_add == dx))) AST_FAIL("%s: bad args", name);
+  hipLaunchKernelGGL((layernorm_bwd_kernel<false, ACC>), dim3((rows + 3) / 4), dim3(256), 0, (hipStream_t)stream, (const float*)dy,
+                     (const float*)x, gamma, mean, rstd, (float*)dx, dgamma, dbeta, rows, D, dx_add);
+  AST_CHECK_LAUNCH();
+  return 0;
+}
+
 extern "C" int ast_layernorm_bwd(const void* dy, const void* x, const float* gamma, const float* mean, const float* rstd,
                                  void* dx, float* dgamma, float* dbeta, int rows, int D, int dtype, void* stream) {
-  if (dtype != AST_F32) AST_FAIL("ast_layernorm_bwd: f32 only");
-  if (!dy || !x || !gamma || !mean || !rstd || !dx || rows <= 0 || D <= 0) AST_FAIL("ast_layernorm_bwd: bad args");
-  hipLaunchKernelGGL(layernorm_bwd_kernel<false>, dim3((rows + 3) / 4), dim3(256), 0, (hipStream_t)stream, (const float*)dy,
-                     (const float*)x, gamma, mean, rstd, (float*)dx, dgamma, dbeta, rows, D);
-  AST_CHECK_LAUNCH();
-  return 0;
+  return layernorm_bwd_launch<false>("ast_layernorm_bwd", dy, x, gamma, mean, rstd, dx, dgamma, dbeta, rows, D, dtype, nullptr, stream);
+}
+
+extern "C" int ast_layernorm_bwd_acc(const void* dy, const void* x, const float* gamma, const float* mean, const float* rstd,
+                                     void* dx, float* dgamma, float* dbeta, int rows, int D, int dtype, const float* dx_add, void* stream) {
+  return layernorm_bwd_launch<true>("ast_layernorm_bwd_acc", dy, x, gamma, mean, rstd, dx, dgamma, dbeta, rows, D, dtype, dx_add, stream);
 }
 
 extern "C" int ast_add_drop_ln_fwd(const float* x, const float* sub, float* mask, float* s_out, const float* gamma, const float* beta,
@@ -893,21 +930,41 @@
   return 0;
 }
 
+static bool adln_adds_ok(const float* dx_add, const float* dsub_add, const float* dx, const float* dsub) {
+  return (dx_add || dsub_add) && !(dx_add && (!dx || dx_add == dx || dx_add == dsub)) && !(dsub_add && (dsub_add == dx || dsub_add == dsub));
+}
+
+template <bool ACC>
+static int add_drop_ln_bwd_launch(const char* name, const float* dy, const float* ds_ext, const float* s, const float* gamma,
+                                  const float* mean, const float* rstd, const float* mask, float* dx, float* dsub, float* dgamma,
+                                  float* dbeta, int rows, int D, const float* dx_add, const float* dsub_add, void* stream) {
+  if ((!dy && !ds_ext) || !dsub || rows <= 0 || D <= 0) AST_FAIL("%s: bad args", name);
+  if (dy && (!s || !gamma || !mean || !rstd)) AST_FAIL("%s: LayerNorm state missing", name);
+  if (ACC && !adln_adds_ok(dx_add, dsub_add, dx, dsub)) AST_FAIL("%s: an addend is missing, has no output or aliases one", name);
+  const bool al = ((((uintptr_t)dy) | ((uintptr_t)ds_ext) | ((uintptr_t)s) | ((uintptr_t)gamma) | ((uintptr_t)mask) | ((uintptr_t)dx) |
+                    ((uintptr_t)dsub) | ((uintptr_t)dx_add) | ((uintptr_t)dsub_add)) & 15) == 0;
+  if (D == 256 && al)
+    hipLaunchKernelGGL(add_drop_ln_bwd256_kernel<ACC>, dim3((rows + 3) / 4), dim3(256), 0, (hipStream_t)stream, dy, ds_ext, s, gamma, mean, rstd,
+                       mask, dx, dsub, dgamma, dbeta, rows, dx_add, dsub_add);
+  else
+    hipLaunchKernelGGL((add_drop_ln_bwd_kernel<false, ACC>), dim3((rows + 3) / 4), dim3(256), 0, (hipStream_t)stream, dy, ds_ext, s, gamma, mean,
+                       rstd, mask, dx, dsub, dgamma, dbeta, rows, D, dx_add, dsub_add);
+  AST_CHECK_LAUNCH();
+  return 0;
+}
+
 extern "C" int ast_add_drop_ln_bwd(const float* dy, const float* ds_ext, const float* s, const float* gamma, const float* mean,
                                    const float* rstd, const float* mask, float* dx, float* dsub, float* dgamma, float* dbeta, int rows,
                                    int D, void* stream) {
-  if ((!dy && !ds_ext) || !dsub || rows <= 0 || D <= 0) AST_FAIL("ast_add_drop_ln_bwd: bad args");
-  if (dy && (!s || !gamma || !mean || !rstd)) AST_FAIL("ast_add_drop_ln_bwd: LayerNorm state missing");
-  const bool al = ((((uintptr_t)dy) | ((uintptr_t)ds_ext) | ((uintptr_t)s) | ((uintptr_t)gamma) | ((uintptr_t)mask) | ((uintptr_t)dx) |
-                    ((uintptr_t)dsub)) & 15) == 0;
-  if (D == 256 && al)
-    hipLaunchKernelGGL(add_drop_ln_bwd256_kernel, dim3((rows + 3) / 4), dim3(256), 0, (hipStream_t)stream, dy, ds_ext, s, gamma, mean, rstd,
-                       mask, dx, dsub, dgamma, dbeta, rows);
-  else
-    hipLaunchKernelGGL(add_drop_ln_bwd_kernel<false>, dim3((rows + 3) / 4), dim3(256), 0, (hipStream_t)stream, dy, ds_ext, s, gamma, mean, rstd,
-                       mask, dx, dsub, dgamma, dbeta, rows, D);
-  AST_CHECK_LAUNCH();
-  return 0;
+  return add_drop_ln_bwd_launch<false>("ast_add_drop_ln_bwd", dy, ds_ext, s, gamma, mean, rstd, mask, dx, dsub, dgamma, dbeta, rows, D, nullptr,
+                                       nullptr, stream);
+}
+
+extern "C" int ast_add_drop_ln_bwd_acc(const float* dy, const float* ds_ext, const float* s, const float* gamma, const float* mean,
+                                       const float* rstd, const float* mask, float* dx, float* dsub, float* dgamma, float* dbeta, int rows,
+                                       int D, const float* dx_add, const float* dsub_add, void* stream) {
+  return add_drop_ln_bwd_launch<true>("ast_add_drop_ln_bwd_acc", dy, ds_ext, s, gamma, mean, rstd, mask, dx, dsub, dgamma, dbeta, rows, D,
+                                      dx_add, dsub_add, stream);
 }
 
 extern "C" int ast_ordered_sum(const float* parts, int64_t n, int nslots, int batches, float* out, int accumulate, void* stream);
@@ -939,30 +996,61 @@
   return ast_ordered_sum(ws, (int64_t)C * 3, nslots, N, sums3, 0, stream);
 }
 
+template <bool ACC>
+static int layernorm_bwd_det_launch(const char* name, const void* dy, const void* x, const float* gamma, const float* mean, const float* rstd,
+                                    void* dx, float* dgamma, float* dbeta, int rows, int D, int dtype, float* ws, const float* dx_add,
+                                    void* stream) {
+  if (dtype != AST_F32) AST_FAIL("%s: f32 only", name);
+  if (!dy || !x || !gamma || !mean || !rstd || !dx || !ws || rows <= 0 || rows > AST_DET_MAX_SLOTS || D <= 0 || (ACC && (!dx_add || dx_add == dx)))
+    AST_FAIL("%s: bad args (1..%d rows)", name, AST_DET_MAX_SLOTS);
+  hipLaunchKernelGGL((layernorm_bwd_kernel<true, ACC>), dim3((rows + 3) / 4), dim3(256), 0, (hipStream_t)stream, (const float*)dy,
+                     (const float*)x, gamma, mean, rstd, (float*)dx, dgamma ? ws : nullptr, dbeta ? ws + (size_t)rows * D : nullptr, rows, D,
+                     dx_add);
+  AST_CHECK_LAUNCH();
+  if (dgamma) if (int rc = ast_ordered_sum(ws, D, rows, 1, dgamma, 1, stream)) return rc;
+  if (dbeta) if (int rc = ast_ordered_sum(ws + (size_t)rows * D, D, rows, 1, dbeta, 1, stream)) return rc;
+  return 0;
+}
+
 extern "C" int ast_layernorm_bwd_det(const void* dy, const void* x, const float* gamma, const float* mean, const float* rstd, void* dx,
                                      float* dgamma, float* dbeta, int rows, int D, int dtype, float* ws, void* stream) {
-  if (dtype != AST_F32) AST_FAIL("ast_layernorm_bwd_det: f32 only");
-  if (!dy || !x || !gamma || !mean || !rstd || !dx || !ws || rows <= 0 || rows > AST_DET_MAX_SLOTS || D <= 0)
-    AST_FAIL("ast_layernorm_bwd_det: bad args (1..%d rows)", AST_DET_MAX_SLOTS);
-  hipLaunchKernelGGL(layernorm_bwd_kernel<true>, dim3((rows + 3) / 4), dim3(256), 0, (hipStream_t)stream, (const float*)dy,
-                     (const float*)x, gamma, mean, rstd, (float*)dx, dgamma ? ws : nullptr, dbeta ? ws + (size_t)rows * D : nullptr, rows, D);
-  AST_CHECK_LAUNCH();
-  if (dgamma) if (int rc = ast_ordered_sum(ws, D, rows, 1, dgamma, 1, stream)) return rc;
-  if (dbeta) if (int rc = ast_ordered_sum(ws + (size_t)rows * D, D, rows, 1, dbeta, 1, stream)) return rc;
+  return layernorm_bwd_det_launch<false>("ast_layernorm_bwd_det", dy, x, gamma, mean, rstd, dx, dgamma, dbeta, rows, D, dtype, ws, nullptr, stream);
+}
+
+extern "C" int ast_layernorm_bwd_det_acc(const void* dy, const void* x, const float* gamma, const float* mean, const float* rstd, void* dx,
+                                         float* dgamma, float* dbeta, int rows, int D, int dtype, float* ws, const float* dx_add, void* stream) {
+  return layernorm_bwd_det_launch<true>("ast_layernorm_bwd_det_acc", dy, x, gamma, mean, rstd, dx, dgamma, dbeta, rows, D, dtype, ws, dx_add,
+                                        stream);
+}
+
+template <bool ACC>
+static int add_drop_ln_bwd_det_launch(const char* name, const float* dy, const float* ds_ext, const float* s, const float* gamma,
+                                      const float* mean, const float* rstd, const float* mask, float* dx, float* dsub, float* dgamma,
+                                      float* dbeta, int rows, int D, float* ws, const float* dx_add, const float* dsub_add, void* stream) {
+  if ((!dy && !ds_ext) || !dsub || rows <= 0 || rows > AST_DET_MAX_SLOTS || D <= 0) AST_FAIL("%s: bad args", name);
+  if (dy && (!s || !gamma || !mean || !rstd)) AST_FAIL("%s: LayerNorm state missing", name);
+  if (ACC && !adln_adds_ok(dx_add, dsub_add, dx, dsub)) AST_FAIL("%s: an addend is missing, has no output or aliases one", name);
+  const bool red = dy && (dgamma || dbeta);
+  if (red && !ws) AST_FAIL("%s: the gamma / beta gradients need 2 * rows * D floats of ws", name);
+  hipLaunchKernelGGL((add_drop_ln_bwd_kernel<true, ACC>), dim3((rows + 3) / 4), dim3(256), 0, (hipStream_t)stream, dy, ds_ext, s, gamma, mean,
+                     rstd, mask, dx, dsub, red && dgamma ? ws : nullptr, red && dbeta ? ws + (size_t)rows * D : nullptr, rows, D, dx_add,
+                     dsub_add);
+  AST_CHECK_LAUNCH();
+  if (red && dgamma) if (int rc = ast_ordered_sum(ws, D, rows, 1, dgamma, 1, stream)) return rc;
+  if (red && dbeta) if (int rc = ast_ordered_sum(ws + (size_t)rows * D, D, rows, 1, dbeta, 1, stream)) return rc;
   return 0;
 }
 
 extern "C" int ast_add_drop_ln_bwd_det(const float* dy, const float* ds_ext, const float* s, const float* gamma, const float* mean,
                                        const float* rstd, const float* mask, float* dx, float* dsub, float* dgamma, float* dbeta, int rows,
                                        int D, float* ws, void* stream) {
-  if ((!dy && !ds_ext) || !dsub || rows <= 0 || rows > AST_DET_MAX_SLOTS || D <= 0) AST_FAIL("ast_add_drop_ln_bwd_det: bad args");
-  if (dy && (!s || !gamma || !mean || !rstd)) AST_FAIL("ast_add_drop_ln_bwd_det: LayerNorm state missing");
-  const bool red = dy && (dgamma || dbeta);
-  if (red && !ws) AST_FAIL("ast_add_drop_ln_bwd_det: the gamma / beta gradients need 2 * rows * D floats of ws");
-  hipLaunchKernelGGL(add_drop_ln_bwd_kernel<true>, dim3((rows + 3) / 4), dim3(256), 0, (hipStream_t)stream, dy, ds_ext, s, gamma, mean, rstd,
-                     mask, dx, dsub, red && dgamma ? ws : nullptr, red && dbeta ? ws + (size_t)rows * D : nullptr, rows, D);
-  AST_CHECK_LAUNCH();
-  if (red && dgamma) if (int rc = ast_ordered_sum(ws, D, rows, 1, dgamma, 1, stream)) return rc;
-  if (red && dbeta) if (int rc = ast_ordered_sum(ws + (size_t)rows * D, D, rows, 1, dbeta, 1, stream)) return rc;
-  return 0;
-}
+  return add_drop_ln_bwd_det_launch<false>("ast_add_drop_ln_bwd_det", dy, ds_ext, s, gamma, mean, rstd, mask, dx, dsub, dgamma, dbeta, rows, D, ws,
+                                           nullptr, nullptr, stream);
+}
+
+extern "C" int ast_add_drop_ln_bwd_det_acc(const float* dy, const float* ds_ext, const float* s, const float* gamma, const float* mean,
+                                           const float* rstd, const float* mask, float* dx, float* dsub, float* dgamma, float* dbeta, int rows,
+                                           int D, float* ws, const float* dx_add, const float* dsub_add, void* stream) {
+  return add_drop_ln_bwd_det_launch<true>("ast_add_drop_ln_bwd_det_acc", dy, ds_ext, s, gamma, mean, rstd, mask, dx, dsub, dgamma, dbeta, rows, D,
+                                          ws, dx_add, dsub_add, stream);
+}
diff --git a/audio-style-transfer_amd/csrc/skinny.hip b/audio-style-transfer_amd/csrc/skinny.hip
--- a/audio-style-transfer_amd/csrc/skinny.hip
+++ b/audio-style-transfer_amd/csrc/skinny.hip
@@ -11,12 +11,16 @@
   return r;
 }
 
-template <int RT, int NS, int NW>
+template <bool ACC> struct SkinnyOut { using Y = float* __restrict__; using A = const float* __restrict__; };
+template <> struct SkinnyOut<true> { using Y = float*; using A = const float*; };
+
+template <int RT, int NS, int NW, bool ACC = false>
 __global__ __launch_bounds__(64 * NW) void skinny_gemm_kernel(const float* __restrict__ x, const float* __restrict__ w,
-                                                           const float* __restrict__ bias, float* __restrict__ y, int M, int N,
+                                                           const float* __restrict__ bias, typename SkinnyOut<ACC>::Y y, int M, int N,
                                                            int K, int ldx, int ldw, int ldy, int relu,
                                                            const float* __restrict__ mul_mask, float* __restrict__ drop_mask,
-                                                           float p, uint64_t seed, const int64_t* __restrict__ d_offset) {
+                                                           float p, uint64_t seed, const int64_t* __restrict__ d_offset,
+                                                           typename SkinnyOut<ACC>::A addend, int ldadd) {
   __shared__ f32x4 part[NW][RT][64];
   const int lane = threadIdx.x & 63, wave = threadIdx.x >> 6;
   const int i = lane & 15, g = lane >> 4;
@@ -39,6 +43,13 @@
   if (bias) {
 #pragma unroll
     for (int q = 0; q < 4; ++q) { const int n = n0 + 4 * g + q; bq[q] = bias[n < N ? n : 0]; }
+  }
+  float aq[4] = {0.f, 0.f, 0.f, 0.f};
+  if (ACC && wave < RT) {
+    const int ma = m0 + 16 * wave + i;
+    const float* ar = addend + (size_t)(ma < M ? ma : 0) * ldadd;
+#pragma unroll
+    for (int q = 0; q < 4; ++q) { const int n = n0 + 4 * g + q; aq[q] = ar[n < N ? n : 0]; }
   }
   f32x4 wl[NS], xl[RT][NS];
 #pragma unroll
@@ -84,6 +95,7 @@
         v *= km;
       }
       if (mul_mask) v *= mul_mask[o];
+      if constexpr (ACC) v = add_rn(v, aq[q]);
       y[o] = v;
     }
   }
@@ -415,10 +427,11 @@
 template <int RT> constexpr int rows_hi() { return RT == 1 ? 64 : AST_WIDE_MAX_ROWS; }
 template <int RT> constexpr bool rows_ok(int M) { return M >= rows_lo<RT>() && M <= rows_hi<RT>(); }
 
-template <int RT>
+template <int RT, bool ACC = false>
 int skinny_gemm_launch(const char* name, const float* x, const float* w, const float* bias, float* y, int M, int N, int K, int ldw,
                        int ldy, int relu, const float* mul_mask, float* drop_mask, float p, uint64_t seed, const int64_t* d_offset,
-                       void* stream) {
+                       void* stream, const float* addend = nullptr, int ldadd = 0) {
+  if (ACC && (!addend || ldadd < N || (((uintptr_t)addend) & 3))) AST_FAIL("%s: addend missing, misaligned or ldadd=%d < N=%d", name, ldadd, N);
   if (!x || !w || !y || !rows_ok<RT>(M) || N < 1 || K < 4 || (K & 3) || (ldw & 3) || (RT > 1 && (ldw < K || ldy < N)))
     AST_FAIL("%s: bad args M=%d (%d..%d) N=%d K=%d ldw=%d ldy=%d", name, M, rows_lo<RT>(), rows_hi<RT>(), N, K, ldw, ldy);
   if ((((uintptr_t)x) | ((uintptr_t)w)) & 15) AST_FAIL("%s: operands must be 16-byte aligned", name);
@@ -426,8 +439,8 @@
   const int steps = (K + 63) / 64;
   if (steps > 16) AST_FAIL("%s: K=%d too large for the token path (<= 1024)", name, K);
   dim3 grid((N + 15) / 16, (M + 16 * RT - 1) / (16 * RT));
-#define AST_SK(NS_, NW_) hipLaunchKernelGGL((skinny_gemm_kernel<RT, NS_, NW_>), grid, dim3(64 * NW_), 0, (hipStream_t)stream, x, w, bias, y, \
-                                            M, N, K, K, ldw, ldy, relu, mul_mask, drop_mask, p, seed, d_offset)
+#define AST_SK(NS_, NW_) hipLaunchKernelGGL((skinny_gemm_kernel<RT, NS_, NW_, ACC>), grid, dim3(64 * NW_), 0, (hipStream_t)stream, x, w, bias, y, \
+                                            M, N, K, K, ldw, ldy, relu, mul_mask, drop_mask, p, seed, d_offset, addend, ldadd)
   if (steps <= 2) AST_SK(2, 4);
   else if (steps <= 4) AST_SK(4, 4);
   else if (steps <= 8) AST_SK(8, 4);
@@ -614,6 +627,20 @@
   return bign_dgrad_launch<4, true>("ast_bign_dgrad_wide_det", dy, w, dx, M, N, K, lddy, ws, ws_floats, stream);
 }
 
+extern "C" int ast_skinny_gemm_acc(const float* x, const float* w, const float* bias, float* y, int M, int N, int K, int ldw, int ldy,
+                                   int relu, const float* mul_mask, float* drop_mask, float p, uint64_t seed, const int64_t* d_offset,
+                                   const float* addend, int ldadd, void* stream) {
+  return skinny_gemm_launch<1, true>("ast_skinny_gemm_acc", x, w, bias, y, M, N, K, ldw, ldy, relu, mul_mask, drop_mask, p, seed, d_offset,
+                                     stream, addend, ldadd);
+}
+
+extern "C" int ast_skinny_gemm_wide_acc(const float* x, const float* w, const float* bias, float* y, int M, int N, int K, int ldw, int ldy,
+                                        int relu, const float* mul_mask, float* drop_mask, float p, uint64_t seed, const int64_t* d_offset,
+                                        const float* addend, int ldadd, void* stream) {
+  return skinny_gemm_launch<4, true>("ast_skinny_gemm_wide_acc", x, w, bias, y, M, N, K, ldw, ldy, relu, mul_mask, drop_mask, p, seed,
+                                     d_offset, stream, addend, ldadd);
+}
+
 extern "C" int ast_bign_gemm_len(const float* x, const float* w, const float* bias, float* y, int M, int N, int K, int ldw, int ldy, int S,
                                  const int32_t* n_valid, void* stream) {
   return bign_gemm_len_launch("ast_bign_gemm_len", x, w, bias, y, M, N, K, ldw, ldy, S, n_valid, stream);
diff --git a/include/ast_hip.h b/include/ast_hip.h
--- a/include/ast_hip.h
+++ b/include/ast_hip.h
@@ -336,6 +336,23 @@
 int ast_bign_dgrad_wide_det(const float* dy, const float* w, float* dx, int M, int N, int K, int lddy, float* ws, long ws_floats,
                             void* stream);
 
+int ast_skinny_gemm_acc(const float* x, const float* w, const float* bias, float* y, int M, int N, int K, int ldw, int ldy, int relu,
+                        const float* mul_mask, float* drop_mask, float p, uint64_t seed, const int64_t* d_offset, const float* addend,
+                        int ldadd, void* stream);
+int ast_skinny_gemm_wide_acc(const float* x, const float* w, const float* bias, float* y, int M, int N, int K, int ldw, int ldy, int relu,
+                             const float* mul_mask, float* drop_mask, float p, uint64_t seed, const int64_t* d_offset,
+                             const float* addend, int ldadd, void* stream);
+int ast_layernorm_bwd_acc(const void* dy, const void* x, const float* gamma, const float* mean, const float* rstd, void* dx,
+                          float* dgamma, float* dbeta, int rows, int D, int dtype, const float* dx_add, void* stream);
+int ast_layernorm_bwd_det_acc(const void* dy, const void* x, const float* gamma, const float* mean, const float* rstd, void* dx,
+                              float* dgamma, float* dbeta, int rows, int D, int dtype, float* ws, const float* dx_add, void* stream);
+int ast_add_drop_ln_bwd_acc(const float* dy, const float* ds_ext, const float* s, const float* gamma, const float* mean,
+                            const float* rstd, const float* mask, float* dx, float* dsub, float* dgamma, float* dbeta, int rows, int D,
+                            const float* dx_add, const float* dsub_add, void* stream);
+int ast_add_drop_ln_bwd_det_acc(const float* dy, const float* ds_ext, const float* s, const float* gamma, const float* mean,
+                                const float* rstd, const float* mask, float* dx, float* dsub, float* dgamma, float* dbeta, int rows,
+                                int D, float* ws, const float* dx_add, const float* dsub_add, void* stream);
+
 #define AST_BIGN_MAX_ROWS 4096
 int ast_bign_gemm_len(const float* x, const float* w, const float* bias, float* y, int M, int N, int K, int ldw, int ldy, int S,
                       const int32_t* n_valid , void* stream);
```
